# Zhen-Dong/HAWQ

Measured on AMD Instinct MI355X. Metric: images/sec, higher is better.
Workload: dtype int8

## Files before the change

### hawq_amd/_lib.py

```python
from __future__ import annotations

import ctypes as C
import os

_HERE = os.path.dirname(os.path.abspath(__file__))
LIB_PATH = os.environ.get("HAWQ_LIB") or os.path.join(_HERE, "lib", "libhawq_mi355.so")

EPI_RAW, EPI_REQUANT, EPI_RESIDUAL, EPI_DEQUANT = 0, 1, 2, 3

i32, i64, f32, vp = C.c_int32, C.c_int64, C.c_float, C.c_void_p


class ConvArgs(C.Structure):
    _fields_ = [
        ("in_", vp), ("wgt", vp), ("bias", vp),
        ("N", i32), ("H", i32), ("W", i32), ("Cin", i32), ("Cout", i32), ("KH", i32), ("KW", i32),
        ("stride", i32), ("pad", i32), ("in_bits", i32), ("w_bits", i32),
        ("in2", vp), ("wgt2", vp), ("bias2", vp),
        ("H2", i32), ("W2", i32), ("Cin2", i32), ("stride2", i32), ("in2_bits", i32), ("w2_bits", i32),
        ("epilogue", i32), ("relu", i32),
        ("m", vp), ("e", vp), ("m_id", vp), ("e_id", vp),
        ("m_id_scalar", i32), ("e_id_scalar", i32),
        ("res_in", vp), ("res_in_bits", i32),
        ("res_out", vp), ("res_out_bits", i32),
        ("out_q", vp), ("out_bits", i32), ("q_lo", i32), ("q_hi", i32), ("mq", i32), ("eq", i32),
        ("out_acc", vp), ("out_f32", vp), ("fscale", vp), ("ldo", i32), ("n_valid", i32),
        ("flags", vp), ("tile", i32), ("ctab", vp), ("ctab_id", vp), ("fast_tables", i32),
        ("in_planar", i32), ("out_planar", i32),
        ("res_no_relu", i32), ("res_clamp16", i32),
        ("in_pitch", i32), ("out_pitch", i32),
        ("wgt_band", vp), ("wgt_k128", vp), ("wgt2_k128", vp),
    ]


class ExpandReduceArgs(C.Structure):
    _fields_ = [("expand", ConvArgs), ("reduce", ConvArgs), ("tile", i32)]


class BottleneckArgs(C.Structure):
    _fields_ = [("expand", ConvArgs), ("project", ConvArgs), ("dw_wgt9c", vp), ("dw_ctab", vp),
                ("dw_stride", i32), ("dw_q_lo", i32), ("dw_q_hi", i32), ("dw_fast_tables", i32), ("c_mid", i32), ("tile", i32)]


class IncepConvArgs(C.Structure):
    _fields_ = [
        ("in_", vp), ("wgt", vp), ("bias", vp),
        ("N", i32), ("H", i32), ("W", i32), ("Cin", i32), ("Cout", i32), ("KH", i32), ("KW", i32),
        ("stride", i32), ("pad_h", i32), ("pad_w", i32),
        ("epilogue", i32), ("relu", i32),
        ("m", vp), ("ek", vp),
        ("q_lo", i32), ("q_hi", i32), ("m2", i32), ("ek2", i32), ("q2_lo", i32), ("q2_hi", i32),
        ("out", vp),
        ("out_bits", i32), ("ldo", i32), ("c_off", i32), ("reserved", i32),
    ]


INCEP_RAW, INCEP_REQUANT, INCEP_REQUANT2 = 0, 1, 2
INCEP_GROUP_MAX = 8


class IncepGroupArgs(C.Structure):
    _fields_ = [("n", i32), ("reserved", i32), ("conv", IncepConvArgs * INCEP_GROUP_MAX)]


INCEP_POOL_OPS = {"hawq_incep_requant": 0, "hawq_incep_maxpool3s2": 1, "hawq_incep_avgpool_branch": 2, "hawq_incep_global_avgpool": 3}


class IncepPoolArgs(C.Structure):
    _fields_ = [("in_", vp), ("out", vp)] + [(n, i32) for n in (
        "N", "H", "W", "C", "in_bits", "in_pitch", "in_off", "out_bits", "ldo", "c_off",
        "pre", "m1", "ek1", "lo1", "hi1", "post", "m2", "ek2", "lo2", "hi2")]


SIGNATURES = {
    "hawq_abi_version": [],
    "hawq_device_ok": [],
    "hawq_conv2d": [C.POINTER(ConvArgs), vp],
    "hawq_conv2d_num_tiles": [],
    "hawq_conv2d_num_band_tiles": [],
    "hawq_conv2d_band_tile": [C.POINTER(ConvArgs)],
    "hawq_conv2d_num_band2_tiles": [],
    "hawq_conv2d_band2_tile": [C.POINTER(ConvArgs)],
    "hawq_pack_w3x3_band": [vp, vp, i32, i32],
    "hawq_conv2d_num_gemm2_tiles": [],
    "hawq_conv2d_gemm2_first": [],
    "hawq_pack_w1x1_k128": [vp, vp, i32, i32],
    "hawq_conv2d_splitk_ok": [C.POINTER(ConvArgs), i32],
    "hawq_conv2d_splitk_workspace": [C.POINTER(ConvArgs), i32, C.POINTER(i64), C.POINTER(i64)],
    "hawq_conv2d_splitk": [C.POINTER(ConvArgs), i32, vp, vp, vp],
    "hawq_fc_dequant_ok": [i32, i32, i32],
    "hawq_fc_dequant": [vp, vp, vp, vp, vp, i32, i32, i32, i32, i32, vp],
    "hawq_conv_expand_reduce": [C.POINTER(ExpandReduceArgs), vp],
    "hawq_conv_expand_reduce_variants": [C.POINTER(ExpandReduceArgs)],
    "hawq_linear_bottleneck": [C.POINTER(BottleneckArgs), vp],
    "hawq_linear_bottleneck_ok": [C.POINTER(BottleneckArgs)],
    "hawq_stem3x3s2": [vp, vp, vp, i32, i32, f32, i32, i32, C.POINTER(ConvArgs), vp],
    "hawq_stem3x3s2_ok": [vp, vp, vp, i32, i32, C.POINTER(ConvArgs)],
    "hawq_quantize_input": [vp, vp, i32, i32, i32, i32, i32, i32, i32, i32, f32, i32, i32, vp],
    "hawq_stem_conv7": [vp, vp, vp, vp, vp, i32, i32, i32, i32, i32, i32, i32, vp, vp, vp],
    "hawq_stem_fused": [vp, i32, i32, i32, i32, f32, i32, i32, vp, vp, vp, vp, i32, i32, vp, vp, i32, i32, i32, i32, i32,
                        i32, vp],
    "hawq_stem_fused_u8": [vp, vp, i32, i32, i32, i32, vp, vp, vp, vp, i32, i32, vp, vp, i32, i32, i32, i32, i32, i32, vp],
    "hawq_maxpool3s2_requant": [vp, i32, i32, i32, i32, vp, vp, i32, i32, i32, i32, i32, vp],
    "hawq_requant_residual": [vp, i32, i64, vp, i32, i32, i32, i32, i32, vp],
    "hawq_avgpool_requant": [vp, i32, i32, i32, i32, vp, vp, i32, i32, i32, i32, vp],
    "hawq_f32_nchw_to_q_nhwc": [vp, vp, i32, i32, i32, i32, i32, i32, f32, vp],
    "hawq_acc_nhwc_to_f32_nchw": [vp, vp, i32, i32, i32, i32, i32, vp, vp],
    "hawq_fixedpoint_f32": [vp, vp, i32, i32, i32, f32, vp, vp, vp, i32, vp, f32, vp, vp, vp, i32, f32, i32, i32,
                            i32, vp],
    "hawq_fakequant_f32": [vp, vp, i64, f32, f32, i32, i32, vp],
    "hawq_avgpool_f32": [vp, vp, i32, i32, f32, vp],
    "hawq_conv2d_grouped": [vp, vp, vp, i32, i32, i32, i32, i32, i32, i32, i32, i32, i32, vp, vp],
    "hawq_depthwise3x3": [vp, vp, vp, i32, i32, i32, i32, i32, vp, vp],
    "hawq_depthwise3x3_requant": [vp, vp, vp, vp, vp, i32, i32, i32, i32, i32, i32, i32, i32, i32, vp, vp, vp],
# ... 77 lines not shown
```

### hawq_amd/csrc/conv_igemm.hip

```cpp
#include <stdio.h>
#include <stdlib.h>

#include "common.h"

namespace {

struct ConvP {
    const uint8_t *in, *wgt;
    const int32_t *bias;
    int N, H, W, Cin, Cout, KH, KW, stride, pad, Ho, Wo, M;
    int in_bits, w_bits;
    const uint8_t *in2, *wgt2;
    const int32_t *bias2;
    int H2, W2, Cin2, stride2, in2_bits, w2_bits;
    int relu;
    const int32_t *m, *e, *m_id, *e_id;
    int m_id_s, e_id_s;
    const void *res_in;
    int res_in_bits;
    void *res_out;
    int res_out_bits;
    void *out_q;
    int out_bits, q_lo, q_hi, mq, eq;
    int32_t *out_acc;
    float *out_f32;
    const float *fscale;
    int ldo, n_valid;
    int32_t *flags;
    const int32_t *ctab, *ctab_id;
    int k0;
    int ck0;
    int res_no_relu, res_clamp16;
    int ring_bytes;
    int in_planar, out_planar;
    int gfast;
    int in_pitch, out_pitch;
    int dbg;
    long long *dbgbuf;
};

template <int BM_, int BN_, int WM_, int WN_, int NS_, int KSUB_ = 1, int MINB_ = 2, int KG_ = 1>
struct Cfg {
    static constexpr int BM = BM_, BN = BN_, WM = WM_, WN = WN_;
    static constexpr int MINB = MINB_;
    static constexpr int NS = NS_;
    static constexpr int KSUB = KSUB_;
    static constexpr int KG = KG_;
    static constexpr int NWG = WM_ * WN_;
    static constexpr int NW = NWG * KG;
    static constexpr int NT = NW * 64;
    static constexpr int NTG = NWG * 64;
    static constexpr int RPP = NTG / 4;
    static constexpr int PT = BM / WM / 32;
    static constexpr int CT = BN / WN / 32;
    static constexpr int AL = BM / RPP;
    static constexpr int WL = BN / RPP;
    static constexpr int STAGE_BYTES = KSUB * (BM + BN) * 64;
    static constexpr int LDS_BYTES = NS * STAGE_BYTES;
    static_assert(NW == 4 || NW == 8 || NW == 16, "4, 8 or 16 waves per workgroup");
    static_assert(BM % RPP == 0 && BN % RPP == 0, "tile rows must fill whole staging passes");
    static_assert(KSUB % KG == 0 && (KG == 1 || BM * BN * 4 <= LDS_BYTES), "split-K: sub-chunks per group, partial sums staged on the ring");
};

template <bool SIGNED16>
__device__ __forceinline__ v4i unpack16(unsigned x0, unsigned x1) {
    v4i r;
    if (SIGNED16) {
        r.x = (int)((x0 << 4) & 0xF0F0F0F0u);
        r.y = (int)(x0 & 0xF0F0F0F0u);
        r.z = (int)((x1 << 4) & 0xF0F0F0F0u);
        r.w = (int)(x1 & 0xF0F0F0F0u);
    } else {
        r.x = (int)(x0 & 0x0F0F0F0Fu);
        r.y = (int)((x0 >> 4) & 0x0F0F0F0Fu);
        r.z = (int)(x1 & 0x0F0F0F0Fu);
        r.w = (int)((x1 >> 4) & 0x0F0F0F0Fu);
    }
    return r;
}

template <int BITS>
__device__ __forceinline__ v4i load_chunk16(const uint8_t *p, bool valid) {
    v4i z = {0, 0, 0, 0};
    if (!valid) return z;
    if (BITS == 8) return *reinterpret_cast<const v4i *>(p);
    v2i t = *reinterpret_cast<const v2i *>(p);
    z.x = t.x;
    z.y = t.y;
    return z;
}

template <class C, int A_BITS, int W_BITS>
__device__ __forceinline__ void gemm_segment(v16i (&acc)[C::CT][C::PT], const uint8_t *__restrict__ in,
                                             const uint8_t *__restrict__ wgt, int H, int W, int Cin, int KH,
                                             int KW, int stride, int pad, int Ho, int Wo, int M, int Cout,
                                             int m0, int c0, char *smem, int apitch) {
    const int t = threadIdx.x;
    const int lane = t & 63, wave = t >> 6;
    const int wave_m = wave % C::WM, wave_c = wave / C::WM;
    const int lrow = t >> 2, lslot = t & 3;
    constexpr int ABYTES = A_BITS == 8 ? 16 : 8;
    constexpr int WBYTES = W_BITS == 8 ? 16 : 8;

    int pix_base[C::AL], iy0[C::AL], ix0[C::AL];
    bool mval[C::AL];
#pragma unroll
    for (int i = 0; i < C::AL; ++i) {
        const int m = m0 + lrow + C::RPP * i;
        mval[i] = m < M;
        const int mm = mval[i] ? m : 0;
        const int n = mm / (Ho * Wo);
        const int r = mm - n * (Ho * Wo);
        const int oy = r / Wo, ox = r - oy * Wo;
        iy0[i] = oy * stride - pad;
        ix0[i] = ox * stride - pad;
        pix_base[i] = (n * H + iy0[i]) * W + ix0[i];
    }
    const int taps = KH * KW;
    const int cchunks = Cin >> 6;
// ... 232 lines not shown
                }
                return;
            }
            const int slot = 2 * (s & 1) + h;
#pragma unroll
            for (int c = 0; c < C::CT; ++c) wf[buf][c] = *reinterpret_cast<const v4i *>(ldsW + lds_off(wrow[c], slot));
#pragma unroll
            for (int q = 0; q < C::PT; ++q) af[buf][q] = *reinterpret_cast<const v4i *>(ldsA + lds_off(arow[q], slot));
        };
        constexpr int NOWN = SPS * KSUB / C::KG;
        auto step_of = [&](int o) { return C::KG == 1 ? o : ((o / SPS) * C::KG + kg) * SPS + (o % SPS); };
        fetch(step_of(0), 0);
#pragma unroll
        for (int o = 0; o < NOWN; ++o) {
            if (o + 1 < NOWN) fetch(step_of(o + 1), (o + 1) & 1);
#pragma unroll
            for (int c = 0; c < C::CT; ++c)
#pragma unroll
                for (int q = 0; q < C::PT; ++q)
                    a[c][q] = __builtin_amdgcn_mfma_i32_32x32x32_i8(wf[o & 1][c], af[o & 1][q], a[c][q], 0, 0, 0);
        }
    };

    const int ns1 = nk1 / KSUB, nst = RANGE ? ke : nk / KSUB;
    const int kfirst = RANGE ? kb : 0;
#pragma unroll
    for (int j = 0; j < NS - 1; ++j)
        if (kfirst + j < nst) issue();
    int cstage = 0;
    constexpr int LS = L * KSUB / C::KG;
    auto step = [&](auto &a, int k) {
        const int after = min(NS - 2, nst - 1 - k);
        if (after >= NS - 2) {
            wait_vmcnt<(NS - 2) * LS>();
        } else {
            switch (after) {
                case 5: wait_vmcnt<(NS > 6 ? 5 : 0) * LS>(); break;
                case 4: wait_vmcnt<(NS > 5 ? 4 : 0) * LS>(); break;
                case 3: wait_vmcnt<(NS > 4 ? 3 : 0) * LS>(); break;
                case 2: wait_vmcnt<(NS > 3 ? 2 : 0) * LS>(); break;
                case 1: wait_vmcnt<(NS > 2 ? 1 : 0) * LS>(); break;
                default: wait_vmcnt<0>(); break;
            }
        }
        __builtin_amdgcn_s_barrier();
        if (jissue < (RANGE ? nst * KSUB : nk) && !HAWQ_DBG_BIT(p.dbg, 1)) issue();
        if (!HAWQ_DBG_BIT(p.dbg, 2)) compute(a, cstage);
        if (++cstage == NS) cstage = 0;
    };
    for (int k = kfirst; k < (RANGE ? min(ns1, nst) : ns1); ++k) step(acc, k);
    if constexpr (DUAL)
        for (int k = RANGE ? max(ns1, kfirst) : ns1; k < nst; ++k) step(acc2, k);
    if constexpr (NIB) {
#pragma unroll
        for (int c = 0; c < C::CT; ++c)
#pragma unroll
            for (int q = 0; q < C::PT; ++q)
#pragma unroll
                for (int r = 0; r < 16; ++r) {
                    acc[c][q][r] >>= 4;
                    if constexpr (DUAL) acc2[DUAL ? c : 0][DUAL ? q : 0][r] >>= 4;
                }
    }
    __syncthreads();
}

template <class C, int BITS>
__device__ __forceinline__ void run_segment(v16i (&acc)[C::CT][C::PT], const uint8_t *in, const uint8_t *wgt,
                                            int a_bits, int w_bits, int H, int W, int Cin, int KH, int KW,
                                            int stride, int pad, int Ho, int Wo, int M, int Cout, int m0, int c0,
                                            char *smem, int apitch) {
    if (BITS == 0x88 || (BITS == 0 && a_bits == 8 && w_bits == 8))
        gemm_segment<C, 8, 8>(acc, in, wgt, H, W, Cin, KH, KW, stride, pad, Ho, Wo, M, Cout, m0, c0, smem, apitch);
    else if (BITS == 0x44 || (BITS == 0 && a_bits == 4 && w_bits == 4))
        gemm_segment<C, 4, 4>(acc, in, wgt, H, W, Cin, KH, KW, stride, pad, Ho, Wo, M, Cout, m0, c0, smem, apitch);
    else if (BITS == 0x84 || (BITS == 0 && a_bits == 8 && w_bits == 4))
        gemm_segment<C, 8, 4>(acc, in, wgt, H, W, Cin, KH, KW, stride, pad, Ho, Wo, M, Cout, m0, c0, smem, apitch);
    else
        gemm_segment<C, 4, 8>(acc, in, wgt, H, W, Cin, KH, KW, stride, pad, Ho, Wo, M, Cout, m0, c0, smem, apitch);
}

__device__ __forceinline__ v4i ld4(const int32_t *p) { return *reinterpret_cast<const v4i *>(p); }


template <class C, int EPI, bool DUAL>
__device__ __forceinline__ void epilogue_generic(const ConvP &p, v16i (&acc)[C::CT][C::PT],
                                                 v16i (&acc2)[DUAL ? C::CT : 1][DUAL ? C::PT : 1], int m0, int c0) {
    const int lane = threadIdx.x & 63, wave = threadIdx.x >> 6;
    const int wave_m = wave % C::WM, wave_c = wave / C::WM;
    const int l31 = lane & 31, h = lane >> 5;
#pragma unroll
    for (int c = 0; c < C::CT; ++c) {
        const int ch = c0 + wave_c * (C::CT * 32) + c * 32 + h * 16;
#pragma unroll
        for (int q = 0; q < C::PT; ++q) {
            const int pix = m0 + wave_m * (C::PT * 32) + q * 32 + l31;
            if (pix >= p.M) continue;
            constexpr bool PITCHED = EPI == HAWQ_EPI_REQUANT || EPI == HAWQ_EPI_RESIDUAL;
            const int opitch = PITCHED ? p.out_pitch : p.Cout;
            const size_t elem = (size_t)pix * opitch + ch;
            bool ovf = false;
            int qw[4] = {0, 0, 0, 0};
#pragma unroll
            for (int g = 0; g < 4; ++g) {
                if (PITCHED && ch + 4 * g >= opitch) continue;
                const v4i b4 = ld4(p.bias + ch + 4 * g);
                const int bb[4] = {b4.x, b4.y, b4.z, b4.w};
                int v[4], qv[4] = {0, 0, 0, 0}, o[4] = {0, 0, 0, 0};
#pragma unroll
                for (int j = 0; j < 4; ++j) v[j] = acc[c][q][4 * g + j] + bb[j];
                if constexpr (EPI == HAWQ_EPI_RAW) {
                    v4i w = {v[0], v[1], v[2], v[3]};
                    reinterpret_cast<v4i *>(p.out_acc + elem)[g] = w;
                } else if constexpr (EPI == HAWQ_EPI_DEQUANT) {
#pragma unroll
                    for (int j = 0; j < 4; ++j)
                        if (ch + 4 * g + j < p.n_valid)
                            p.out_f32[(size_t)pix * p.ldo + ch + 4 * g + j] = (float)v[j] * p.fscale[ch + 4 * g + j];
                } else if (p.n_valid > 0 && ch + 4 * g >= p.n_valid) {
                    if (EPI == HAWQ_EPI_RESIDUAL && p.res_out) {
                        if (p.res_out_bits == 16) reinterpret_cast<v2i *>((uint16_t *)p.res_out + elem)[g] = v2i{0, 0};
                        else reinterpret_cast<v4i *>((int32_t *)p.res_out + elem)[g] = v4i{0, 0, 0, 0};
                    }
                    if ((EPI == HAWQ_EPI_REQUANT || p.out_q) && p.out_bits == 4 && !(g & 1)) reinterpret_cast<uint32_t *>((uint8_t *)p.out_q + (elem >> 1) + (g >> 1) * 4)[0] = 0u;
                } else if (EPI == HAWQ_EPI_RESIDUAL && !DUAL && p.gfast) {
                    const bool tie = p.k0 == 2;
                    const DyNt dids = dynt_prepare(p.m_id_s, p.e_id_s), dq = dynt_prepare(p.mq, p.eq);
#pragma unroll
                    for (int j = 0; j < 4; ++j) {
                        const v4i t4 = ld4(p.ctab + (size_t)(ch + 4 * g + j) * 4);
                        DyNt dm;
                        dm.m = t4.x, dm.s = t4.y & 31, dm.k = t4.y >> 8;
                        dm.add = (long long)(((unsigned long long)(unsigned)t4.w << 32) | (unsigned)t4.z);
                        const int av = acc[c][q][4 * g + j];
                        int ov = tie ? dyadic_tie(av, dm) : dyadic_nt(av, dm);
                        if (p.res_in) {
                            const int r = p.res_in_bits == 16 ? (int)((const uint16_t *)p.res_in)[elem + 4 * g + j]
                                                              : ((const int32_t *)p.res_in)[elem + 4 * g + j];
                            ov += tie ? dyadic_tie(r, dids) : dyadic_nt(r, dids);
                        }
                        if (!p.res_no_relu) ov = max(ov, 0);
                        if (p.res_clamp16) ov = clampi(ov, -32768, 32767);
                        o[j] = ov;
                        qv[j] = clampi(tie ? dyadic_tie(ov, dq) : dyadic_nt(ov, dq), p.q_lo, p.q_hi);
                        ovf |= ov > 65535;
                    }
                    if (p.res_out) {
                        if (p.res_out_bits == 16) {
                            v2i w = {min(o[0], 65535) | (min(o[1], 65535) << 16), min(o[2], 65535) | (min(o[3], 65535) << 16)};
                            reinterpret_cast<v2i *>((uint16_t *)p.res_out + elem)[g] = w;
                        } else {
                            v4i w = {o[0], o[1], o[2], o[3]};
                            reinterpret_cast<v4i *>((int32_t *)p.res_out + elem)[g] = w;
                        }
                    }
                    if (p.out_q) {
                        if (p.out_bits == 8) {
                            qw[g] = (int)pack4_i8(qv[0], qv[1], qv[2], qv[3]);
                        } else {
                            uint8_t *dst = (uint8_t *)p.out_q + (elem >> 1) + (g >> 1) * 4;
#pragma unroll
                            for (int j = 0; j < 4; ++j) dst[j] = (g & 1) ? (uint8_t)((dst[j] & 0x0f) | (qv[j] << 4)) : (uint8_t)(qv[j] & 0x0f);
                        }
                    }
                } else {
                    const v4i m4 = ld4(p.m + ch + 4 * g), e4 = ld4(p.e + ch + 4 * g);
                    const int mm[4] = {m4.x, m4.y, m4.z, m4.w}, ee[4] = {e4.x, e4.y, e4.z, e4.w};
                    if constexpr (EPI == HAWQ_EPI_REQUANT) {
#pragma unroll
                        for (int j = 0; j < 4; ++j)
                            qv[j] = clampi(dyadic_rne(p.relu ? max(v[j], 0) : v[j], mm[j], ee[j]), p.q_lo, p.q_hi);
                    } else {
                        int idv[4];
                        if constexpr (DUAL) {
                            const v4i b2 = ld4(p.bias2 + ch + 4 * g), mi = ld4(p.m_id + ch + 4 * g),
                                      ei = ld4(p.e_id + ch + 4 * g);
                            const int bb2[4] = {b2.x, b2.y, b2.z, b2.w}, m1[4] = {mi.x, mi.y, mi.z, mi.w},
                                      e1[4] = {ei.x, ei.y, ei.z, ei.w};
#pragma unroll
                            for (int j = 0; j < 4; ++j) idv[j] = dyadic_rne(acc2[DUAL ? c : 0][DUAL ? q : 0][4 * g + j] + bb2[j], m1[j], e1[j]);
                        } else if (p.res_in) {
#pragma unroll
                            for (int j = 0; j < 4; ++j) {
                                const int r = p.res_in_bits == 16 ? (int)((const uint16_t *)p.res_in)[elem + 4 * g + j]
                                                                  : ((const int32_t *)p.res_in)[elem + 4 * g + j];
                                idv[j] = dyadic_rne(r, p.m_id_s, p.e_id_s);
                            }
                        } else {
#pragma unroll
                            for (int j = 0; j < 4; ++j) idv[j] = 0;
                        }
#pragma unroll
                        for (int j = 0; j < 4; ++j) {
                            o[j] = dyadic_rne(v[j], mm[j], ee[j]) + idv[j];
                            if (!p.res_no_relu) o[j] = max(o[j], 0);
                            if (p.res_clamp16) o[j] = clampi(o[j], -32768, 32767);
                            qv[j] = clampi(dyadic_rne(o[j], p.mq, p.eq), p.q_lo, p.q_hi);
                            ovf |= o[j] > 65535;
                        }
                        if (p.res_out) {
                            if (p.res_out_bits == 16) {
                                v2i w = {min(o[0], 65535) | (min(o[1], 65535) << 16), min(o[2], 65535) | (min(o[3], 65535) << 16)};
                                reinterpret_cast<v2i *>((uint16_t *)p.res_out + elem)[g] = w;
                            } else {
                                v4i w = {o[0], o[1], o[2], o[3]};
                                reinterpret_cast<v4i *>((int32_t *)p.res_out + elem)[g] = w;
                            }
                        }
                    }
                    if (EPI == HAWQ_EPI_REQUANT || p.out_q) {
                        if (p.out_bits == 8) {
                            qw[g] = (int)pack4_i8(qv[0], qv[1], qv[2], qv[3]);
                        } else {
                            uint8_t *dst = (uint8_t *)p.out_q + (elem >> 1) + (g >> 1) * 4;
                            if (g & 1) {
#pragma unroll
                                for (int j = 0; j < 4; ++j) dst[j] = (uint8_t)((dst[j] & 0x0f) | (qv[j] << 4));
                            } else {
#pragma unroll
                                for (int j = 0; j < 4; ++j) dst[j] = (uint8_t)(qv[j] & 0x0f);
                            }
                        }
                    }
                }
            }
            if constexpr (PITCHED) {
                if ((EPI == HAWQ_EPI_REQUANT || p.out_q) && p.out_bits == 8 && ch < opitch)
                    *reinterpret_cast<v4i *>((char *)p.out_q + elem) = v4i{qw[0], qw[1], qw[2], qw[3]};
            }
            if (EPI == HAWQ_EPI_RESIDUAL && ovf && p.res_out && p.res_out_bits == 16) atomicOr(p.flags, 1);
        }
    }
}

template <class C>
struct Stage {
    static constexpr int RCPR = C::BN / 8;
    static constexpr int QCPR = C::BN / 16;
    __device__ static __forceinline__ int rsw(int row) { return row & (RCPR - 1); }
    __device__ static __forceinline__ int qsw(int row) {
        return QCPR >= 8 ? (row & (QCPR - 1)) : ((row >> 1) & (QCPR - 1));
    }
};

template <class C>
__device__ __forceinline__ void prefetch_residual(const ConvP &p, int m0, int c0, char *res_tile) {
    using S = Stage<C>;
    const int wave = threadIdx.x >> 6, lane = threadIdx.x & 63;
#pragma unroll
    for (int i = 0; i < (C::BM * S::RCPR + C::NT - 1) / C::NT; ++i) {
        const int base = (i * C::NW + wave) * 64;
        if (base >= C::BM * S::RCPR) break;
        const int idx = base + lane;
        const int row = idx / S::RCPR, j = idx % S::RCPR;
        const int grow = (m0 + row < p.M) ? m0 + row : m0;
        const char *src = (const char *)p.res_in + ((size_t)grow * p.Cout + c0) * 2 + ((j ^ S::rsw(row)) << 4);
        __builtin_amdgcn_global_load_lds((const __attribute__((address_space(1))) void *)src,
                                         (__attribute__((address_space(3))) void *)(res_tile + base * 16), 16, 0, 0);
    }
}

template <class C, int EPI, bool DUAL, int MODE = 0, bool CK0 = false>
__device__ __forceinline__ void epilogue_fast(const ConvP &p, v16i (&acc)[C::CT][C::PT],
                                              v16i (&acc2)[DUAL ? C::CT : 1][DUAL ? C::PT : 1], int m0, int c0,
                                              char *q_tile, char *res_tile, const char *ctab_lds,
                                              const bool active = true) {
    using S = Stage<C>;
    constexpr bool RES = EPI == HAWQ_EPI_RESIDUAL;
    constexpr bool K0 = MODE == 1 || CK0;
    constexpr int MODE_C = (CK0 && MODE == 0) ? 1 : MODE;
    const int lane = threadIdx.x & 63, wave = threadIdx.x >> 6;
    const int wave_m = wave % C::WM, wave_c = (wave / C::WM) % C::WN;
    const int l31 = lane & 31, h = lane >> 5;
    const int lrow0 = wave_m * (C::PT * 32) + l31;
    DyNt dids = dynt_prepare(p.m_id_s, p.e_id_s), dq = dynt_prepare(p.mq, p.eq);
    asm volatile("" : "+s"(dids.add), "+s"(dq.add));
    const int qhi2 = (p.q_hi & 0xffff) | (p.q_hi << 16);
    unsigned oor = 0;
    unsigned rowmask[C::PT];
#pragma unroll
    for (int q = 0; q < C::PT; ++q) rowmask[q] = (m0 + lrow0 + q * 32 < p.M) ? 0xffffffffu : 0u;
    if (active)
#pragma unroll
    for (int c = 0; c < C::CT; ++c) {
        const int lch = wave_c * (C::CT * 32) + c * 32 + h * 16;
        constexpr int WPS = (C::NT / 256 > C::MINB) ? C::NT / 256 : C::MINB;
        constexpr int QPASS = (DUAL || (RES && WPS >= 4)) ? C::PT : 1, QPER = C::PT / QPASS;
#pragma unroll
        for (int qp = 0; qp < QPASS; ++qp) {
        v4i rin[C::PT][2];
        if constexpr (RES && !DUAL) {
#pragma unroll
            for (int qq = 0; qq < QPER; ++qq) {
                const int q = qp * QPER + qq;
                const int row = lrow0 + q * 32;
                const char *base = res_tile + row * (S::RCPR * 16);
                rin[q][0] = *reinterpret_cast<const v4i *>(base + (((lch >> 3) ^ S::rsw(row)) << 4));
                rin[q][1] = *reinterpret_cast<const v4i *>(base + ((((lch >> 3) + 1) ^ S::rsw(row)) << 4));
            }
        }
        int qpack[QPER][4];
        int rpack[QPER][RES ? 8 : 1];
#pragma unroll
        for (int g = 0; g < 4; ++g) {
            DyNt dm[4], di[4];
#pragma unroll
            for (int j = 0; j < 4; ++j) {
                const v4i t = *reinterpret_cast<const v4i *>(ctab_lds + (lch + 4 * g + j) * 16);
                dm[j].m = t.x, dm[j].s = K0 ? t.y : (t.y & 31), dm[j].k = K0 ? 0 : (t.y >> 8);
                dm[j].add = (long long)(((unsigned long long)(unsigned)t.w << 32) | (unsigned)t.z);
                if constexpr (DUAL) {
                    const v4i u = *reinterpret_cast<const v4i *>(ctab_lds + C::BN * 16 + (lch + 4 * g + j) * 16);
                    di[j].m = u.x, di[j].s = K0 ? u.y : (u.y & 31), di[j].k = K0 ? 0 : (u.y >> 8);
                    di[j].add = (long long)(((unsigned long long)(unsigned)u.w << 32) | (unsigned)u.z);
                } else {
                    di[j] = dids;
                }
            }
#pragma unroll
            for (int qq = 0; qq < QPER; ++qq) {
                const int q = qp * QPER + qq;
                int qv[4];
                if constexpr (!RES) {
#pragma unroll
                    for (int j = 0; j < 4; ++j)
                        qv[j] = med3i(dyadic_mode<MODE_C>(acc[c][q][4 * g + j], dm[j]), p.q_lo, p.q_hi);
                } else {
                    int idin[4], o[4];
                    if constexpr (DUAL) {
#pragma unroll
                        for (int j = 0; j < 4; ++j) idin[j] = acc2[DUAL ? c : 0][DUAL ? q : 0][4 * g + j];
                    } else {
                        const unsigned w0 = (unsigned)rin[q][g >> 1][(g & 1) * 2], w1 = (unsigned)rin[q][g >> 1][(g & 1) * 2 + 1];
                        idin[0] = (int)(w0 & 0xffffu), idin[1] = (int)(w0 >> 16);
                        idin[2] = (int)(w1 & 0xffffu), idin[3] = (int)(w1 >> 16);
                    }
#pragma unroll
                    for (int j = 0; j < 4; ++j) {
                        const int a = dyadic_mode<MODE_C>(acc[c][q][4 * g + j], dm[j]);
// ... 441 lines not shown
        BAND_FETCH(0, 0)
        for (int s = 0; s < nsteps; ++s) {
            BAND_BATCH(0)
            if (C::NPROD == 0 && early && !HAWQ_DBG_BIT(p.dbg, 1)) issue_step(s, cc, kh);
            BAND_BATCH(1)
            BAND_BATCH(2)
            BAND_BATCH(3)
            if (C::NPROD == 0 && !early && !HAWQ_DBG_BIT(p.dbg, 1)) issue_step(s, cc, kh);
            BAND_BATCH(4)
            if (++kh == 3) kh = 0, ++cc;
            if (s + 1 < nsteps) {
                bases(s + 1, cc, kh);
                BAND_FETCH(0, 0)
                wait_lgkm<C::CT + C::PT>();
            } else {
                wait_lgkm<0>();
            }
            BAND_MMA(5)
            if (C::NPROD == 0) wait_vmcnt<0>();
            __builtin_amdgcn_s_barrier();
        }
#undef BAND_FETCH
#undef BAND_MMA
#undef BAND_BATCH
        if (C::NPROD > 0) __builtin_amdgcn_s_setprio(0);
    }
    const long long t_loop_end = prof ? (long long)__builtin_readcyclecounter() : 0;
    if constexpr (NIB) {
#pragma unroll
        for (int c = 0; c < C::CT; ++c)
#pragma unroll
            for (int q = 0; q < C::PT; ++q)
#pragma unroll
                for (int r = 0; r < 16; ++r) acc[c][q][r] >>= 4;
    }
    __syncthreads();
    if constexpr (EPI == HAWQ_EPI_RESIDUAL) {
        using S = Stage<C>;
        static_assert(C::BM * C::BN * 2 <= C::WS * C::WSTAGE && C::BM * C::BN <= C::BSTAGES * C::BAND_BYTES, "epilogue tiles alias the rings");
        constexpr int NWALL = C::NT / 64, PPW = C::BM * S::RCPR / 64 / NWALL;
        static_assert(PPW * NWALL * 64 == C::BM * S::RCPR, "residual tile pieces");
#pragma unroll
        for (int i = 0; i < PPW; ++i) {
            const int base = (i * NWALL + wave) * 64, idx = base + lane;
            const int row = idx / S::RCPR, j = idx % S::RCPR;
            const int grow = (m0 + row < p.M) ? m0 + row : m0;
            const char *src = (const char *)p.res_in + ((size_t)grow * p.Cout + c0) * 2 + ((j ^ S::rsw(row)) << 4);
            __builtin_amdgcn_global_load_lds((const __attribute__((address_space(1))) void *)src,
                                             (__attribute__((address_space(3))) void *)(wring + base * 16), 16, 0, 0);
        }
        wait_vmcnt<0>();
        __syncthreads();
    }
    v16i dummy[1][1];
    epilogue_fast<C, EPI, false, TIE ? 2 : 0>(p, acc, dummy, m0, c0, smem, wring, ctab_lds, consumer);
    if (prof && blockIdx.x == 8 && t == 0) {
        p.dbgbuf[0] = t_begin - t_entry, p.dbgbuf[1] = t_loop_end - t_begin;
        p.dbgbuf[2] = (long long)__builtin_readcyclecounter() - t_loop_end, p.dbgbuf[3] = nsteps;
    }
}

using B0 = BandCfg<256, 64, 4, 1, 512, 1, 2, 0>;
using B1 = BandCfg<256, 128, 4, 2, 512, 2, 1, 8>;
using B2 = BandCfg<128, 128, 2, 4, 256, 2, 1, 8, 4>;
using B3 = BandCfg<256, 128, 4, 2, 384, 2, 1, 8, 4>;
using B4 = BandCfg<128, 128, 2, 4, 256, 2, 1, 8, 5>;
using B5 = BandCfg<128, 64, 2, 2, 256, 2, 4, 4, 3>;
constexpr int NUM_BAND_TILES = 6;

typedef void (*KernelFn)(const ConvP);
struct BandInfo { KernelFn fn[2][2][2]; int bm, bn, band_px, bstages, lds, nt; };
#define BAND_FN(B, N, T) {conv3x3_band_kernel<B, N, T, HAWQ_EPI_REQUANT>, conv3x3_band_kernel<B, N, T, HAWQ_EPI_RESIDUAL>}
#define BAND_ENTRY(B) {{{BAND_FN(B, false, false), BAND_FN(B, false, true)}, {BAND_FN(B, true, false), BAND_FN(B, true, true)}}, B::BM, B::BN, B::BAND_PX, B::BSTAGES, B::LDS_BYTES + B::BN * 16, B::NT}
const BandInfo kBand[NUM_BAND_TILES] = {BAND_ENTRY(B0), BAND_ENTRY(B1), BAND_ENTRY(B2), BAND_ENTRY(B3), BAND_ENTRY(B4), BAND_ENTRY(B5)};
const int kBandPreference[NUM_BAND_TILES] = {0, 3, 1, 2, 4, 5};

bool band_applies(const BandInfo &bi, const hawq_conv_args *a) {
    const int wo = a->W, band_rows = (bi.bm + wo - 1) / wo + 1 + 2;
    const bool nib = a->in_bits == 4 && a->w_bits == 4;
    const bool res = a->epilogue == HAWQ_EPI_RESIDUAL;
    const bool epi_ok = (a->epilogue == HAWQ_EPI_REQUANT && a->out_q) ||
                        (res && a->res_in && a->res_in_bits == 16 && (!a->res_out || a->res_out_bits == 16));
    const bool dense = (a->in_pitch == 0 || a->in_pitch == a->Cin * a->in_bits / 8) && (a->out_pitch == 0 || a->out_pitch == a->Cout);
    return a->KH == 3 && a->KW == 3 && a->stride == 1 && a->pad == 1 && a->in2 == nullptr && a->fast_tables != 0 && epi_ok && dense &&
           ((a->in_bits == 8 && a->w_bits == 8) || (nib && a->Cin % 128 == 0)) && a->Cout % bi.bn == 0 &&
           band_rows * (wo + 2) <= bi.band_px - 4 && (bi.bstages > 1 || (a->Cin >> (nib ? 7 : 6)) == 1);
}

using T0 = Cfg<128, 128, 2, 2, 3>;
using T1 = Cfg<256, 64, 4, 1, 3>;
using T2 = Cfg<64, 64, 2, 2, 4>;
using T3 = Cfg<128, 64, 2, 2, 4>;
using T4 = Cfg<128, 128, 2, 2, 3, 2>;
using T5 = Cfg<64, 64, 2, 2, 4, 2>;
using T6 = Cfg<128, 64, 2, 2, 3, 2>;
using T7 = Cfg<128, 128, 2, 4, 3>;
using T8 = Cfg<128, 128, 2, 4, 3, 2>;
using T9 = Cfg<256, 128, 4, 2, 3>;
using T10 = Cfg<64, 64, 2, 2, 3, 1, 6>;
using T11 = Cfg<64, 64, 2, 2, 2, 1, 6>;
using T12 = Cfg<128, 64, 2, 2, 2, 1, 3>;
using T13 = Cfg<128, 128, 2, 4, 2, 1, 2>;
using T14 = Cfg<64, 64, 2, 2, 3, 2, 4, 2>;
constexpr int NUM_TILES = 15;

struct TileInfo {
    int BM, BN, lds, ksub, twin, nt, ns, kg;
    KernelFn single[4][3];
    KernelFn dual[5];
    KernelFn tie_single[2][2];
    KernelFn tie_dual[2];
};
#define SINGLE_ROW(T, E) \
    { conv_kernel<T, E, false, 0, 0>, conv_kernel<T, E, false, 0x88, 0>, conv_kernel<T, E, false, 0x44, 0> }
#define TILE_ENTRY(T, TWIN)                                                                                          \
    {                                                                                                          \
        T::BM, T::BN, T::LDS_BYTES, T::KSUB, TWIN, T::NT, T::NS, T::KG,                                                   \
            {SINGLE_ROW(T, HAWQ_EPI_RAW), SINGLE_ROW(T, HAWQ_EPI_REQUANT), SINGLE_ROW(T, HAWQ_EPI_RESIDUAL),   \
             SINGLE_ROW(T, HAWQ_EPI_DEQUANT)},                                                                 \
        {                                                                                                      \
            conv_kernel<T, HAWQ_EPI_RESIDUAL, true, 0, 0>, conv_kernel<T, HAWQ_EPI_RESIDUAL, true, 0x88, 0x88>, \
                conv_kernel<T, HAWQ_EPI_RESIDUAL, true, 0x44, 0x44>,                                           \
                conv_kernel<T, HAWQ_EPI_RESIDUAL, true, 0x88, 0x44>,                                           \
                conv_kernel<T, HAWQ_EPI_RESIDUAL, true, 0x44, 0x88>                                            \
        },                                                                                                     \
        {{conv_kernel<T, HAWQ_EPI_REQUANT, false, 0x88, 0, true>, conv_kernel<T, HAWQ_EPI_REQUANT, false, 0x44, 0, true>},   \
         {conv_kernel<T, HAWQ_EPI_RESIDUAL, false, 0x88, 0, true>, conv_kernel<T, HAWQ_EPI_RESIDUAL, false, 0x44, 0, true>}}, \
        {conv_kernel<T, HAWQ_EPI_RESIDUAL, true, 0x88, 0x88, true>, conv_kernel<T, HAWQ_EPI_RESIDUAL, true, 0x44, 0x44, true>} \
    }
const TileInfo kTiles[NUM_TILES] = {TILE_ENTRY(T0, 0), TILE_ENTRY(T1, 1), TILE_ENTRY(T2, 2), TILE_ENTRY(T3, 3),
                                    TILE_ENTRY(T4, 0), TILE_ENTRY(T5, 2), TILE_ENTRY(T6, 3),
                                    TILE_ENTRY(T7, 7), TILE_ENTRY(T8, 7), TILE_ENTRY(T9, 9),
                                    TILE_ENTRY(T10, 10), TILE_ENTRY(T11, 11), TILE_ENTRY(T12, 12), TILE_ENTRY(T13, 13),
                                    TILE_ENTRY(T14, 2)};

bool raise_lds_limits() {
    bool ok = true;
    for (const TileInfo &ti : kTiles) {
        const int lds = ti.lds + ti.BM * ti.BN * 2 + ti.BN * 32;
        if (lds <= 64 * 1024) continue;
        for (int v = 0; v < 2; ++v)
            ok &= hipFuncSetAttribute((const void *)ti.tie_single[1][v], hipFuncAttributeMaxDynamicSharedMemorySize, lds) == hipSuccess &&
                  hipFuncSetAttribute((const void *)ti.tie_dual[v], hipFuncAttributeMaxDynamicSharedMemorySize, lds) == hipSuccess;
        for (int v = 1; v < 3; ++v)
            ok &= hipFuncSetAttribute((const void *)ti.single[2][v], hipFuncAttributeMaxDynamicSharedMemorySize, lds) ==
                  hipSuccess;
        for (int v = 1; v < 5; ++v)
            ok &= hipFuncSetAttribute((const void *)ti.dual[v], hipFuncAttributeMaxDynamicSharedMemorySize, lds) ==
                  hipSuccess;
    }
    return ok;
}

int pick_tile(int M, int Cout, bool dual) {
    auto nwg = [&](int t) { return ((M + kTiles[t].BM - 1) / kTiles[t].BM) * (Cout / kTiles[t].BN); };
    if (dual) return nwg(3) >= 512 ? 3 : 2;
    if (Cout % 128 == 0 && nwg(0) >= 1024) return 0;
    if (nwg(1) >= 1024 && !dual) return 1;
    if (Cout % 128 == 0 && nwg(0) >= 512) return 0;
    if (nwg(3) >= 512) return 3;
    return 2;
}

#endif
}
#ifndef HAWQ_CONV_IGEMM_DEVICE_ONLY

bool band_persist_applies(const hawq_conv_args *a);
int band_persist_launch(const hawq_conv_args *a, int exact_tie, int dbg, int wgs_per_cu, void *stream);

int gemm_v2_count(void);
bool gemm_v2_applies(const hawq_conv_args *a, int v);
int gemm_v2_launch(const hawq_conv_args *a, int v, int exact_tie, int dbg, void *stream);
int band_v2_count(void);
bool band_v2_applies(const hawq_conv_args *a, int v);
int band_v2_launch(const hawq_conv_args *a, int v, int exact_tie, int dbg, void *stream);

extern "C" int hawq_conv2d_num_tiles(void) { return NUM_TILES + NUM_BAND_TILES + 2 + band_v2_count() + gemm_v2_count(); }
extern "C" int hawq_conv2d_num_gemm2_tiles(void) { return gemm_v2_count(); }
extern "C" int hawq_conv2d_gemm2_first(void) { return NUM_TILES + NUM_BAND_TILES + 2 + band_v2_count() + 1; }
extern "C" int hawq_conv2d_num_band_tiles(void) { return NUM_BAND_TILES + 2 + band_v2_count() + gemm_v2_count(); }

extern "C" int hawq_conv2d_num_band2_tiles(void) { return band_v2_count(); }
extern "C" int hawq_conv2d_band2_tile(const hawq_conv_args *a) {
    if (!a || a->W <= 0 || a->H <= 0 || a->Cin <= 0 || a->Cout <= 0) return 0;
    for (int v = 0; v < band_v2_count(); ++v)
        if (band_v2_applies(a, v)) return NUM_TILES + NUM_BAND_TILES + 2 + v + 1;
    return 0;
}

extern "C" int hawq_conv2d_band_tile(const hawq_conv_args *a) {
    if (!a || a->W <= 0 || a->H <= 0 || a->Cin <= 0 || a->Cout <= 0) return 0;
    for (int k = 0; k < NUM_BAND_TILES; ++k)
        if (band_applies(kBand[kBandPreference[k]], a)) return NUM_TILES + kBandPreference[k] + 1;
    return 0;
}

extern "C" int hawq_conv2d(const hawq_conv_args *a, void *stream) {
    HAWQ_REQUIRE(a != nullptr, "hawq_conv2d: null args");
    HAWQ_REQUIRE(a->in && a->wgt && a->bias, "hawq_conv2d: in/wgt/bias must be non-null");
    HAWQ_REQUIRE(a->Cin > 0 && a->Cin % 64 == 0, "hawq_conv2d: Cin=%d must be a positive multiple of 64", a->Cin);
    HAWQ_REQUIRE(a->Cout > 0 && a->Cout % 64 == 0, "hawq_conv2d: Cout=%d must be a positive multiple of 64", a->Cout);
    HAWQ_REQUIRE((a->in_bits == 8 || a->in_bits == 4) && (a->w_bits == 8 || a->w_bits == 4),
                 "hawq_conv2d: in_bits/w_bits must be 4 or 8 (got %d/%d)", a->in_bits, a->w_bits);
    HAWQ_REQUIRE(a->KH > 0 && a->KW > 0 && a->stride > 0 && a->pad >= 0 && a->N > 0 && a->H > 0 && a->W > 0,
                 "hawq_conv2d: bad geometry");
    ConvP p;
    p.in = (const uint8_t *)a->in;
    p.wgt = (const uint8_t *)a->wgt;
    p.bias = a->bias;
    p.N = a->N, p.H = a->H, p.W = a->W, p.Cin = a->Cin, p.Cout = a->Cout;
    p.KH = a->KH, p.KW = a->KW, p.stride = a->stride, p.pad = a->pad;
    p.Ho = (a->H + 2 * a->pad - a->KH) / a->stride + 1;
    p.Wo = (a->W + 2 * a->pad - a->KW) / a->stride + 1;
    HAWQ_REQUIRE(p.Ho > 0 && p.Wo > 0, "hawq_conv2d: empty output");
    const long long M = (long long)a->N * p.Ho * p.Wo;
    HAWQ_REQUIRE(M * (long long)a->Cout < (1ll << 40) && M < (1ll << 30), "hawq_conv2d: problem too large");
    p.M = (int)M;
    p.in_bits = a->in_bits, p.w_bits = a->w_bits;
    const bool dual = a->in2 != nullptr;
    p.in2 = (const uint8_t *)a->in2, p.wgt2 = (const uint8_t *)a->wgt2, p.bias2 = a->bias2;
    p.H2 = a->H2, p.W2 = a->W2, p.Cin2 = a->Cin2, p.stride2 = a->stride2;
    p.in2_bits = a->in2_bits, p.w2_bits = a->w2_bits;
    if (dual) {
        HAWQ_REQUIRE(a->epilogue == HAWQ_EPI_RESIDUAL, "hawq_conv2d: second branch needs HAWQ_EPI_RESIDUAL");
        HAWQ_REQUIRE(a->wgt2 && a->bias2 && a->m_id && a->e_id, "hawq_conv2d: second branch tables missing");
        HAWQ_REQUIRE(a->Cin2 > 0 && a->Cin2 % 64 == 0, "hawq_conv2d: Cin2 must be a multiple of 64");
        HAWQ_REQUIRE((a->in2_bits == 8 || a->in2_bits == 4) && (a->w2_bits == 8 || a->w2_bits == 4),
                     "hawq_conv2d: in2_bits/w2_bits must be 4 or 8");
        HAWQ_REQUIRE((a->H2 - 1) / a->stride2 + 1 == p.Ho && (a->W2 - 1) / a->stride2 + 1 == p.Wo,
                     "hawq_conv2d: second branch output grid differs");
    }
    p.relu = a->relu;
    p.m = a->m, p.e = a->e, p.m_id = a->m_id, p.e_id = a->e_id;
    p.m_id_s = a->m_id_scalar, p.e_id_s = a->e_id_scalar;
    p.res_in = a->res_in, p.res_in_bits = a->res_in_bits;
    p.res_no_relu = a->res_no_relu, p.res_clamp16 = a->res_clamp16;
    p.res_out = a->res_out, p.res_out_bits = a->res_out_bits;
    p.out_q = a->out_q, p.out_bits = a->out_bits, p.q_lo = a->q_lo, p.q_hi = a->q_hi, p.mq = a->mq, p.eq = a->eq;
    p.out_acc = a->out_acc, p.out_f32 = a->out_f32, p.fscale = a->fscale, p.ldo = a->ldo, p.n_valid = a->n_valid;
    {
        const int dense_in = a->Cin * a->in_bits / 8;
        p.in_pitch = a->in_pitch ? a->in_pitch : dense_in, p.out_pitch = a->out_pitch ? a->out_pitch : a->Cout;
        if (p.in_pitch != dense_in)
            HAWQ_REQUIRE(a->in_pitch > 0 && a->in_pitch % 16 == 0 && a->in_pitch < dense_in && a->in_bits == 8 && !a->in_planar,
                         "hawq_conv2d: in_pitch=%d needs a multiple of 16 below the dense row (%d bytes), int8 activations, NHWC rows", a->in_pitch, dense_in);
        if (p.out_pitch != a->Cout) {
            const bool fast_ = a->fast_tables != 0;
            HAWQ_REQUIRE(a->out_pitch > 0 && a->out_pitch % 16 == 0 && a->out_pitch < a->Cout, "hawq_conv2d: out_pitch=%d needs a multiple of 16 below Cout=%d", a->out_pitch, a->Cout);
            HAWQ_REQUIRE((a->epilogue == HAWQ_EPI_REQUANT || a->epilogue == HAWQ_EPI_RESIDUAL) && !a->in2 && !a->out_planar && (!a->out_q || a->out_bits == 8),
                         "hawq_conv2d: out_pitch exists for single-branch REQUANT / RESIDUAL launches with int8 NHWC outputs");
            const bool direct_ = a->epilogue == HAWQ_EPI_RESIDUAL &&
                                 (a->res_no_relu || a->res_clamp16 || !a->res_in || a->res_in_bits == 32 || (a->res_out && a->res_out_bits == 32));
            HAWQ_REQUIRE(!fast_ || a->epilogue == HAWQ_EPI_REQUANT || direct_,
                         "hawq_conv2d: out_pitch with fast_tables needs the REQUANT epilogue or a signed / 32-bit RESIDUAL (the unsigned 16-bit fast RESIDUAL tiles are dense)");
            HAWQ_REQUIRE(a->n_valid <= a->out_pitch, "hawq_conv2d: n_valid=%d exceeds out_pitch=%d", a->n_valid, a->out_pitch);
        }
    }
    p.flags = a->flags;
    p.ctab = a->ctab, p.ctab_id = a->ctab_id;
    static const int dbg_env = HAWQ_DBG_ENV();
    p.dbg = a->fast_tables ? dbg_env : 0;
    p.dbgbuf = nullptr;
    static long long *dbg_dev = nullptr;
    if (HAWQ_DBG_BIT(p.dbg, 128) && !dbg_dev) (void)hipMalloc(&dbg_dev, 64 * sizeof(long long));
    if (HAWQ_DBG_BIT(p.dbg, 128)) p.dbgbuf = dbg_dev;
    const bool fast = a->fast_tables != 0;
    p.k0 = (a->fast_tables & 4) ? 2 : ((a->fast_tables & 2) ? 1 : 0);
    p.ck0 = (a->fast_tables & 8) != 0;
    if (fast && (a->epilogue == HAWQ_EPI_REQUANT || a->epilogue == HAWQ_EPI_RESIDUAL)) {
        HAWQ_REQUIRE(a->ctab && (!dual || a->ctab_id), "hawq_conv2d: fast_tables needs ctab (and ctab_id)");
        if (a->epilogue == HAWQ_EPI_REQUANT && a->relu && p.q_lo < 0) p.q_lo = 0;
        const bool direct_form = a->epilogue == HAWQ_EPI_RESIDUAL && !dual &&
                                 (a->res_no_relu || a->res_clamp16 || !a->res_in || a->res_in_bits == 32 || (a->res_out && a->res_out_bits == 32));
        HAWQ_REQUIRE(a->epilogue != HAWQ_EPI_RESIDUAL || !a->out_q || a->q_lo <= 0 || direct_form,
                     "hawq_conv2d: fast RESIDUAL needs q_lo <= 0");
    }
    auto e_fast = [](int ek) { return (ek & 0xff) >= 33 && (ek & 0xff) <= 62; };
    auto e_any = [](int ek) { return (ek & 0xff) >= 1 && (ek & 0xff) <= 62 && (ek >> 8) >= 0 && (ek >> 8) < 31; };
    if (a->epilogue == HAWQ_EPI_RESIDUAL) {
        if (a->out_q) {
            HAWQ_REQUIRE(a->mq >= 0 && e_any(a->eq), "hawq_conv2d: bad (mq, eq)");
            HAWQ_REQUIRE(!fast || e_fast(a->eq), "hawq_conv2d: fast_tables needs eq in [33,62]");
            HAWQ_REQUIRE(!fast || (a->q_hi >= 0 && a->q_hi <= 32767), "hawq_conv2d: fast_tables needs 0 <= q_hi <= 32767 for the next QuantAct");
            HAWQ_REQUIRE(p.k0 != 1 || (a->eq >> 8) == 0, "hawq_conv2d: fast_tables bit 1 (no pre-shifts) but eq carries one");
        } else {
            p.mq = 0, p.eq = 33;
        }
        if (!dual && !a->res_in) {
            p.m_id_s = 0, p.e_id_s = 33;
        } else if (!dual) {
            HAWQ_REQUIRE(a->m_id_scalar >= 0 && e_any(a->e_id_scalar), "hawq_conv2d: bad (m_id_scalar, e_id_scalar)");
            HAWQ_REQUIRE(!fast || e_fast(a->e_id_scalar), "hawq_conv2d: fast_tables needs e_id_scalar in [33,62]");
        } else {
            p.m_id_s = 0, p.e_id_s = 33;
        }
    } else {
        p.mq = 0, p.eq = 33, p.m_id_s = 0, p.e_id_s = 33;
    }
    int slot = -1;
// ... 155 lines not shown
```

### hawq_amd/csrc/conv_splitk.hip

```cpp
#define HAWQ_CONV_IGEMM_DEVICE_ONLY
#include "conv_igemm.hip"

namespace {

using SK = Cfg<64, 64, 2, 2, 4>;
constexpr int SK_TILE = SK::BM * SK::BN;
constexpr int SK_RES = SK::BM * SK::BN * 2;
constexpr int SK_CTAB = SK::BN * 16 * 2;
constexpr int SK_LDS = SK::LDS_BYTES + SK_RES + SK_CTAB + 16;

struct SplitP {
    int32_t *slab;
    int32_t *counters;
    int tiles_c, ntiles;
    int s1, s2;
    int q1, q2;
    int ns1;
};

template <int EPI, bool DUAL, bool FAST, bool TIE, bool PLANAR>
__global__ __launch_bounds__(SK::NT, SK::MINB) void conv_splitk_kernel(const ConvP p, const SplitP s) {
    using C = SK;
    extern __shared__ __attribute__((aligned(16))) char smem[];
    const int tile = blockIdx.x % s.ntiles, z = blockIdx.x / s.ntiles;
// ... 3 lines not shown

    v16i acc[C::CT][C::PT], acc2[C::CT][C::PT];
#pragma unroll
    for (int r = 0; r < 16; ++r) acc[0][0][r] = 0;
    const int kb = z < s.s1 ? z * s.q1 : s.ns1 + (z - s.s1) * s.q2;
    const int ke = kb + (z < s.s1 ? s.q1 : s.q2);
    gemm_pipeline<C, DUAL, false, true, PLANAR>(acc, acc, p, m0, c0, smem, kb, ke);

    const size_t tile_base = (size_t)tile * nsl * SK_TILE;
    int32_t *mine = s.slab + tile_base + (size_t)z * SK_TILE + wave * 1024;
#pragma unroll
    for (int g = 0; g < 4; ++g)
        reinterpret_cast<v4i *>(mine)[g * 64 + lane] = v4i{acc[0][0][4 * g], acc[0][0][4 * g + 1], acc[0][0][4 * g + 2], acc[0][0][4 * g + 3]};
    __builtin_amdgcn_fence(__ATOMIC_RELEASE, "agent");
    __syncthreads();
    int *last = reinterpret_cast<int *>(smem + SK_LDS - 16);
    if (threadIdx.x == 0) {
        const int arrived = __hip_atomic_fetch_add(s.counters + tile, 1, __ATOMIC_RELAXED, __HIP_MEMORY_SCOPE_AGENT);
        *last = arrived == nsl - 1;
    }
    __syncthreads();
    if (!*last) return;
    __builtin_amdgcn_fence(__ATOMIC_ACQUIRE, "agent");
    if (threadIdx.x == 0) s.counters[tile] = 0;

#pragma unroll
    for (int r = 0; r < 16; ++r) acc[0][0][r] = 0, acc2[0][0][r] = 0;
    const int32_t *base = s.slab + tile_base + wave * 1024;
    for (int j = 0; j < s.s1; ++j) {
#pragma unroll
        for (int g = 0; g < 4; ++g) {
            const v4i v = reinterpret_cast<const v4i *>(base + (size_t)j * SK_TILE)[g * 64 + lane];
            acc[0][0][4 * g] += v.x, acc[0][0][4 * g + 1] += v.y, acc[0][0][4 * g + 2] += v.z, acc[0][0][4 * g + 3] += v.w;
        }
    }
    if constexpr (DUAL) {
        for (int j = s.s1; j < nsl; ++j) {
#pragma unroll
            for (int g = 0; g < 4; ++g) {
                const v4i v = reinterpret_cast<const v4i *>(base + (size_t)j * SK_TILE)[g * 64 + lane];
                acc2[0][0][4 * g] += v.x, acc2[0][0][4 * g + 1] += v.y, acc2[0][0][4 * g + 2] += v.z, acc2[0][0][4 * g + 3] += v.w;
            }
        }
    }

    if constexpr (FAST) {
        char *res_tile = smem + p.ring_bytes;
        char *ctab_lds = res_tile + (EPI == HAWQ_EPI_RESIDUAL ? SK_RES : 0);
        if (wave < C::BN / 64)
            __builtin_amdgcn_global_load_lds((const __attribute__((address_space(1))) void *)(p.ctab + (size_t)(c0 + wave * 64 + lane) * 4),
                                             (__attribute__((address_space(3))) void *)(ctab_lds + wave * 1024), 16, 0, 0);
        if constexpr (DUAL) {
            if (wave >= C::NW / 2 && wave - C::NW / 2 < C::BN / 64)
                __builtin_amdgcn_global_load_lds(
                    (const __attribute__((address_space(1))) void *)(p.ctab_id + (size_t)(c0 + (wave - C::NW / 2) * 64 + lane) * 4),
                    (__attribute__((address_space(3))) void *)(ctab_lds + C::BN * 16 + (wave - C::NW / 2) * 1024), 16, 0, 0);
        }
        if constexpr (EPI == HAWQ_EPI_RESIDUAL && !DUAL) prefetch_residual<C>(p, m0, c0, res_tile);
        wait_vmcnt<0>();
        __syncthreads();
        epilogue_fast<C, EPI, DUAL, TIE ? 2 : 0>(p, acc, acc2, m0, c0, smem, res_tile, ctab_lds);
    } else {
        epilogue_generic<C, EPI, DUAL>(p, acc, acc2, m0, c0);
    }
}

typedef void (*SplitFn)(const ConvP, const SplitP);

struct SplitPlan {
    int s1, s2, q1, q2, ns1, tiles_c, ntiles, M, Ho, Wo;
    long long slab_bytes, counter_bytes;
};

int splitk_plan(const hawq_conv_args *a, int slices, SplitPlan &sp) {
    HAWQ_REQUIRE(a != nullptr, "hawq_conv2d_splitk: null args");
    HAWQ_REQUIRE(slices >= 2, "hawq_conv2d_splitk: slices=%d (at least 2)", slices);
    HAWQ_REQUIRE(a->Cin > 0 && a->Cin % 64 == 0 && a->Cout > 0 && a->Cout % 64 == 0, "hawq_conv2d_splitk: Cin / Cout must be positive multiples of 64");
    HAWQ_REQUIRE(a->N > 0 && a->H > 0 && a->W > 0, "hawq_conv2d_splitk: bad geometry");
    HAWQ_REQUIRE(a->in_bits == 8 && a->w_bits == 8, "hawq_conv2d_splitk: int8 operands only (in_bits %d, w_bits %d)", a->in_bits, a->w_bits);
    const bool k1 = a->KH == 1 && a->KW == 1 && a->pad == 0, k3 = a->KH == 3 && a->KW == 3 && a->pad == 1;
    HAWQ_REQUIRE((k1 || k3) && (a->stride == 1 || a->stride == 2), "hawq_conv2d_splitk: 1x1 / pad 0 or 3x3 / pad 1 convs with stride 1 or 2 only");
    HAWQ_REQUIRE(a->n_valid == 0 && (a->in_pitch == 0 || a->in_pitch == a->Cin) && (a->out_pitch == 0 || a->out_pitch == a->Cout),
                 "hawq_conv2d_splitk: n_valid / in_pitch / out_pitch are not supported");
    const int epi = a->epilogue;
    HAWQ_REQUIRE(epi == HAWQ_EPI_RAW || epi == HAWQ_EPI_REQUANT || epi == HAWQ_EPI_RESIDUAL, "hawq_conv2d_splitk: RAW, REQUANT or RESIDUAL epilogue only");
    HAWQ_REQUIRE(epi == HAWQ_EPI_RAW || !a->out_q || a->out_bits == 8, "hawq_conv2d_splitk: out_bits must be 8");
    HAWQ_REQUIRE(epi != HAWQ_EPI_REQUANT || a->out_q, "hawq_conv2d_splitk: REQUANT needs out_q");
    HAWQ_REQUIRE((a->in_planar | a->out_planar | 1) == 1, "hawq_conv2d_splitk: in_planar / out_planar must be 0 or 1");
    const bool dual = a->in2 != nullptr;
    const bool fast = a->fast_tables != 0;
    const bool res = epi == HAWQ_EPI_RESIDUAL;
    const bool wide_res = res && ((!dual && a->res_in_bits == 32) || (a->res_out && a->res_out_bits == 32));
    const bool signed_res = res && !dual && (a->res_no_relu || a->res_clamp16 || !a->res_in);
    const bool fast_epi = fast && epi != HAWQ_EPI_RAW && !wide_res && !signed_res;
    HAWQ_REQUIRE(!a->in_planar || (!dual && fast_epi), "hawq_conv2d_splitk: in_planar needs a single-branch fast-contract REQUANT / RESIDUAL launch");
    HAWQ_REQUIRE(!a->out_planar || (fast_epi && a->out_q), "hawq_conv2d_splitk: out_planar needs the fast-contract REQUANT / RESIDUAL epilogue");
    sp.Ho = (a->H + 2 * a->pad - a->KH) / a->stride + 1;
    sp.Wo = (a->W + 2 * a->pad - a->KW) / a->stride + 1;
    const long long M = (long long)a->N * sp.Ho * sp.Wo;
    HAWQ_REQUIRE(sp.Ho > 0 && sp.Wo > 0 && M < (1ll << 30) && M * (long long)a->Cout < (1ll << 40), "hawq_conv2d_splitk: bad output size");
    sp.M = (int)M;
    const int nk1 = a->KH * a->KW * (a->Cin >> 6);
    HAWQ_REQUIRE(nk1 % slices == 0, "hawq_conv2d_splitk: %d slices do not divide the %d K chunks", slices, nk1);
    sp.s1 = slices, sp.q1 = nk1 / slices, sp.ns1 = nk1, sp.s2 = 0, sp.q2 = 1;
    if (dual) {
        HAWQ_REQUIRE(res, "hawq_conv2d_splitk: a second branch needs HAWQ_EPI_RESIDUAL");
        HAWQ_REQUIRE(a->in2_bits == 8 && a->w2_bits == 8, "hawq_conv2d_splitk: int8 operands only in the second branch");
        HAWQ_REQUIRE(a->Cin2 > 0 && a->Cin2 % 64 == 0 && a->stride2 > 0 && a->H2 > 0 && a->W2 > 0, "hawq_conv2d_splitk: bad second branch");
        HAWQ_REQUIRE((a->H2 - 1) / a->stride2 + 1 == sp.Ho && (a->W2 - 1) / a->stride2 + 1 == sp.Wo, "hawq_conv2d_splitk: second branch output grid differs");
        const int nk2 = a->Cin2 >> 6;
        int q2 = sp.q1 < nk2 ? sp.q1 : nk2;
        while (nk2 % q2) --q2;
        sp.q2 = q2, sp.s2 = nk2 / q2;
    }
    sp.tiles_c = a->Cout / SK::BN;
    sp.ntiles = ((sp.M + SK::BM - 1) / SK::BM) * sp.tiles_c;
    HAWQ_REQUIRE((long long)sp.ntiles * (sp.s1 + sp.s2) < (1ll << 31), "hawq_conv2d_splitk: grid too large");
    sp.slab_bytes = (long long)sp.ntiles * (sp.s1 + sp.s2) * SK_TILE * 4;
    sp.counter_bytes = (long long)sp.ntiles * 4;
    return 0;
}

#define SK_FN(E, D, F, T, P) conv_splitk_kernel<E, D, F, T, P>
SplitFn pick_kernel(int epi, bool dual, bool fast, bool tie, bool planar) {
    if (epi == HAWQ_EPI_RAW) return SK_FN(HAWQ_EPI_RAW, false, false, false, false);
    if (dual) {
        if (!fast) return SK_FN(HAWQ_EPI_RESIDUAL, true, false, false, false);
        return tie ? SK_FN(HAWQ_EPI_RESIDUAL, true, true, true, false) : SK_FN(HAWQ_EPI_RESIDUAL, true, true, false, false);
    }
    if (epi == HAWQ_EPI_REQUANT) {
        if (!fast) return SK_FN(HAWQ_EPI_REQUANT, false, false, false, false);
        if (planar) return tie ? SK_FN(HAWQ_EPI_REQUANT, false, true, true, true) : SK_FN(HAWQ_EPI_REQUANT, false, true, false, true);
        return tie ? SK_FN(HAWQ_EPI_REQUANT, false, true, true, false) : SK_FN(HAWQ_EPI_REQUANT, false, true, false, false);
    }
    if (!fast) return SK_FN(HAWQ_EPI_RESIDUAL, false, false, false, false);
    if (planar) return tie ? SK_FN(HAWQ_EPI_RESIDUAL, false, true, true, true) : SK_FN(HAWQ_EPI_RESIDUAL, false, true, false, true);
    return tie ? SK_FN(HAWQ_EPI_RESIDUAL, false, true, true, false) : SK_FN(HAWQ_EPI_RESIDUAL, false, true, false, false);
}

}

extern "C" int hawq_conv2d_splitk_ok(const hawq_conv_args *a, int32_t slices) {
    SplitPlan sp;
    return splitk_plan(a, slices, sp) == 0 ? 1 : 0;
}

extern "C" int hawq_conv2d_splitk_workspace(const hawq_conv_args *a, int32_t slices, int64_t *slab_bytes, int64_t *counter_bytes) {
    SplitPlan sp;
    const int rc = splitk_plan(a, slices, sp);
    if (rc) return rc;
    if (slab_bytes) *slab_bytes = sp.slab_bytes;
    if (counter_bytes) *counter_bytes = sp.counter_bytes;
    return 0;
}

extern "C" int hawq_conv2d_splitk(const hawq_conv_args *a, int32_t slices, void *slab, int32_t *counters, void *stream) {
    SplitPlan sp;
    const int rc = splitk_plan(a, slices, sp);
    if (rc) return rc;
    HAWQ_REQUIRE(slab && counters, "hawq_conv2d_splitk: slab and counters must be non-null");
    HAWQ_REQUIRE(a->in && a->wgt && a->bias, "hawq_conv2d_splitk: in/wgt/bias must be non-null");
    const bool dual = a->in2 != nullptr;
    const int epi = a->epilogue;
    const bool fast = a->fast_tables != 0;
    ConvP p = {};
    p.in = (const uint8_t *)a->in, p.wgt = (const uint8_t *)a->wgt, p.bias = a->bias;
// ... 65 lines not shown
```

### hawq_amd/csrc/fused_er.hip

```cpp
#include <stdio.h>
#include <stdlib.h>

#include "common.h"

namespace {

struct ERP {
    const uint8_t *x2, *w3, *w1;
    const uint8_t *xid, *wid;
    const int32_t *ctab3, *ctab1, *ctab_id;
    const uint16_t *res_in;
    uint16_t *res_out;
    uint8_t *y;
    int M, C3;
    int m_id_s, e_id_s, mq, eq, q_hi;
    int y_lo, y_hi;
    int y_planar;
    int y_nib;
    int32_t *flags;
    int dbg;
    long long *dbgbuf;
};

__device__ __attribute__((aligned(16))) const int g_er_zero16[4] = {0, 0, 0, 0};
// ... 298 lines not shown
            __syncthreads();
            if (p.y_planar) {
                for (int idx = t; idx < F::BM * CPN; idx += F::NTC) {
                    const int ch = idx / F::BM, row = idx % F::BM;
                    if (m0 + row < p.M)
                        *reinterpret_cast<v4i *>((char *)p.y + ((size_t)ch * p.M + (m0 + row)) * 16) =
                            *reinterpret_cast<const v4i *>(yt + (row * CPN + (ch ^ (row & (CPN - 1)))) * 16);
                }
            } else {
                for (int idx = t; idx < F::BM * CPN; idx += F::NTC) {
                    const int row = idx / CPN, jj = idx % CPN;
                    if (m0 + row < p.M)
                        *reinterpret_cast<v4i *>((char *)p.y + (size_t)(m0 + row) * (F::C / 2) + ((jj ^ (row & (CPN - 1))) << 4)) =
                            *reinterpret_cast<const v4i *>(yt + idx * 16);
                }
            }
            return;
        }
#pragma unroll
        for (int c = 0; c < F::CT2; ++c) {
            const int ch0 = wave_c * (F::CT2 * 32) + c * 32 + h * 16;
            int w[4];
#pragma unroll
            for (int g = 0; g < 4; ++g) {
                int qv[4];
#pragma unroll
                for (int k = 0; k < 4; ++k)
                    qv[k] = med3i(dyadic_mode<MODE_C>(acc2[c][4 * g + k], ctab_entry<K0>((const char *)p.ctab1, ch0 + 4 * g + k)), p.y_lo, p.y_hi);
                w[g] = pack4_fast(qv[0], qv[1], qv[2], qv[3]);
            }
            const v4i ww = {w[0], w[1], w[2], w[3]};
            *reinterpret_cast<v4i *>(yt + (arow * CPR + ((ch0 >> 4) ^ (arow & (CPR - 1)))) * 16) = ww;
        }
        __syncthreads();
        if (p.y_planar) {
#pragma unroll
            for (int i = 0; i < F::BM * CPR / F::NTC; ++i) {
                const int idx = t + F::NTC * i, ch = idx / F::BM, row = idx % F::BM;
                if (m0 + row < p.M)
                    *reinterpret_cast<v4i *>((char *)p.y + ((size_t)ch * p.M + (m0 + row)) * 16) =
                        *reinterpret_cast<const v4i *>(yt + (row * CPR + (ch ^ (row & (CPR - 1)))) * 16);
            }
        } else {
#pragma unroll
            for (int i = 0; i < F::BM * CPR / F::NTC; ++i) {
                const int idx = t + F::NTC * i, row = idx / CPR, jj = idx % CPR;
                if (m0 + row < p.M)
                    *reinterpret_cast<v4i *>((char *)p.y + (size_t)(m0 + row) * F::C + ((jj ^ (row & (CPR - 1))) << 4)) =
                        *reinterpret_cast<const v4i *>(yt + idx * 16);
            }
        }
    }
}

using E64 = ERCfg<64, 2, 0, true, 4>;
using E64R = ERCfg<64, 2, 0, false, 4>;
using E128 = ERCfg<128, 2, 0, false, 3>;
using E128D = ERCfg<128, 2, 0, true, 3>;
using E128P = ERCfg<128, 2, 4, true, 4>;
using E256 = ERCfg<256, 4, 0, false, 2>;
using E256P = ERCfg<256, 4, 4, true, 3>;
using E256S = ERCfg<256, 2, 0, false, 2>;
using E256SP = ERCfg<256, 2, 4, true, 2>;
using E64D = ERCfg<64, 2, 0, false, 4, true>;
constexpr int NUM_ER = 10;

typedef void (*ERFn)(const ERP);
struct ERInfo { ERFn fn[5]; int c, bm, nt, lds; bool dual; };
#define ER_ENTRY(F) {{expand_reduce_kernel<F, false>, expand_reduce_kernel<F, true>, expand_reduce_kernel<F, false, true>, expand_reduce_kernel<F, false, true, true>, \
                      expand_reduce_kernel<F, false, false, true>}, F::C, F::BM, F::NT, F::LDS_BYTES, F::DUAL}
const ERInfo kER[NUM_ER] = {ER_ENTRY(E64), ER_ENTRY(E64R), ER_ENTRY(E128), ER_ENTRY(E128D), ER_ENTRY(E128P), ER_ENTRY(E256), ER_ENTRY(E256P), ER_ENTRY(E256S), ER_ENTRY(E256SP), ER_ENTRY(E64D)};

bool conv_is_1x1_int8_fast(const hawq_conv_args &a, bool dual_ok = false) {
    return (a.in_pitch == 0 || a.in_pitch == a.Cin) && (a.out_pitch == 0 || a.out_pitch == a.Cout) && a.KH == 1 && a.KW == 1 && a.stride == 1 && a.pad == 0 && a.in_bits == 8 && a.w_bits == 8 && a.fast_tables != 0 &&
           (dual_ok || !a.in2) && !a.in_planar;
}

bool dual_branch_fits(const hawq_conv_args &e) {
    return e.in2 && e.wgt2 && e.ctab_id && e.Cin2 == e.Cin && e.stride2 == 1 && e.H2 == e.H && e.W2 == e.W && e.in2_bits == 8 && e.w2_bits == 8;
}

int er_variant(const hawq_expand_reduce_args *a) {
    const hawq_conv_args &e = a->expand, &r = a->reduce;
    if (!conv_is_1x1_int8_fast(e, true) || !conv_is_1x1_int8_fast(r)) return -1;
    const bool dual = e.in2 != nullptr;
    if (dual && !dual_branch_fits(e)) return -1;
    if (e.epilogue != HAWQ_EPI_RESIDUAL || r.epilogue != HAWQ_EPI_REQUANT) return -1;
    if (!dual && (!e.res_in || e.res_in_bits != 16)) return -1;
    if (!e.res_out || e.res_out_bits != 16 || !e.flags || !e.ctab || !r.ctab || !r.out_q) return -1;
    if ((r.out_bits != 8 && r.out_bits != 4) || e.out_bits != 8) return -1;
    if (r.out_bits == 4 && (r.q_lo < 0 || r.q_hi > 15)) return -1;
    if (r.Cin != e.Cout || r.Cout != e.Cin || r.N != e.N || r.H != e.H || r.W != e.W || e.Cout % 64) return -1;
    int nth = 0, first = -1;
    for (int i = 0; i < NUM_ER; ++i)
        if (kER[i].c == e.Cin && kER[i].dual == dual) {
            if (first < 0) first = i;
            if (++nth == a->tile) return i;
        }
    return a->tile == 0 ? first : -1;
}

}

int wp_num_variants(const hawq_expand_reduce_args *a);
int wp_launch(const hawq_expand_reduce_args *a, int nth, void *stream);
int er2_num_variants(const hawq_expand_reduce_args *a);
int er2_launch(const hawq_expand_reduce_args *a, int nth, void *stream);

namespace {
int er_count(const hawq_expand_reduce_args *a) {
    if (!a->reduce.wgt) return 0;
    hawq_expand_reduce_args q = *a;
    q.tile = 0;
    if (er_variant(&q) < 0) return 0;
    int n = 0;
    for (int i = 0; i < NUM_ER; ++i) n += kER[i].c == a->expand.Cin && kER[i].dual == (a->expand.in2 != nullptr);
    return n;
}
}

extern "C" int hawq_conv_expand_reduce_variants(const hawq_expand_reduce_args *a) {
    if (!a) return 0;
    return er_count(a) + wp_num_variants(a) + er2_num_variants(a);
}

extern "C" int hawq_conv_expand_reduce(const hawq_expand_reduce_args *a, void *stream) {
    HAWQ_REQUIRE(a != nullptr, "hawq_conv_expand_reduce: null args");
    const int n_er = er_count(a), n_wp = wp_num_variants(a);
    if (a->tile > n_er + n_wp) return er2_launch(a, a->tile - n_er - n_wp, stream);
    if (a->tile > n_er || (a->tile == 0 && n_er == 0)) return wp_launch(a, a->tile == 0 ? 1 : a->tile - n_er, stream);
    const int v = er_variant(a);
    HAWQ_REQUIRE(v >= 0, "hawq_conv_expand_reduce: this pair of layers cannot be fused (need 1x1/stride-1 int8 fast-contract convs, "
                         "uint16 residual in and out - or a same-shape 1x1 identity branch with Cin 64 -, Cin in {64,128,256}, reduce.Cin == expand.Cout, reduce.Cout == expand.Cin; tile %d)", a->tile);
    const hawq_conv_args &e = a->expand, &r = a->reduce;
    auto e_fast = [](int ek) { return (ek & 0xff) >= 33 && (ek & 0xff) <= 62; };
    HAWQ_REQUIRE(e.mq >= 0 && e_fast(e.eq) && (e.in2 || (e.m_id_scalar >= 0 && e_fast(e.e_id_scalar))), "hawq_conv_expand_reduce: scalar tables outside the fast contract");
    HAWQ_REQUIRE(e.q_lo <= 0, "hawq_conv_expand_reduce: the block-input QuantAct clamp must admit 0");
    ERP p;
    p.x2 = (const uint8_t *)e.in, p.w3 = (const uint8_t *)e.wgt, p.w1 = (const uint8_t *)r.wgt;
    p.ctab3 = e.ctab, p.ctab1 = r.ctab;
    p.xid = (const uint8_t *)e.in2, p.wid = (const uint8_t *)e.wgt2, p.ctab_id = e.ctab_id;
    p.res_in = (const uint16_t *)e.res_in, p.res_out = (uint16_t *)e.res_out;
    p.y = (uint8_t *)r.out_q;
    const long long M = (long long)e.N * e.H * e.W;
    HAWQ_REQUIRE(M > 0 && M < (1ll << 30), "hawq_conv_expand_reduce: bad problem size");
    p.M = (int)M, p.C3 = e.Cout;
    p.m_id_s = e.in2 ? 0 : e.m_id_scalar, p.e_id_s = e.in2 ? 33 : e.e_id_scalar, p.mq = e.mq, p.eq = e.eq, p.q_hi = e.q_hi;
    p.y_lo = r.relu && r.q_lo < 0 ? 0 : r.q_lo, p.y_hi = r.q_hi;
    p.y_planar = r.out_planar;
    p.y_nib = r.out_bits == 4;
    p.flags = e.flags;
    static const int dbg_env = HAWQ_DBG_ENV();
    static long long *dbg_dev = nullptr;
    if (HAWQ_DBG_BIT(dbg_env, 128) && !dbg_dev) (void)hipMalloc(&dbg_dev, 64 * sizeof(long long));
    p.dbgbuf = HAWQ_DBG_BIT(dbg_env, 128) ? dbg_dev : nullptr;
    p.dbg = dbg_env;
    const ERInfo &ei = kER[v];
    static const bool attrs = [] {
        bool good = true;
        for (const ERInfo &k : kER)
            for (int i = 0; i < 5; ++i)
                good &= hipFuncSetAttribute((const void *)k.fn[i], hipFuncAttributeMaxDynamicSharedMemorySize, k.lds) == hipSuccess;
        return good;
    }();
    HAWQ_REQUIRE(attrs, "hawq_conv_expand_reduce: hipFuncSetAttribute(MaxDynamicSharedMemorySize) failed");
    const bool tie = ((e.fast_tables | r.fast_tables) & 4) != 0, ck0 = (e.fast_tables & 8) && (r.fast_tables & 8);
    const bool qk0 = (e.eq >> 8) == 0;
// ... 14 lines not shown
```

### hawq_amd/csrc/fused_er2.hip

```cpp
#include <stdio.h>
#include <stdlib.h>

#include "common.h"

namespace {

struct E2P {
    const uint8_t *x2, *w3, *w1;
    const int32_t *ctab3, *ctab1;
    const uint16_t *res_in;
    uint16_t *res_out;
    uint8_t *y;
    int M, C3;
    int m_id_s, e_id_s, mq, eq, q_hi;
    int y_lo, y_hi;
    int y_planar, y_nib;
    int32_t *flags;
    long long *dbgbuf;
    int dbg;
};

__device__ __attribute__((aligned(16))) const int g_e2_zero16[4] = {0, 0, 0, 0};

template <int C_, int WM_, int NP_, int MINB_, int SG_ = 4>
// ... 260 lines not shown
            constexpr int CPN = F::C / 32;
#pragma unroll
            for (int c = 0; c < F::CT2; ++c) {
                const int ch0 = wave_c * (F::CT2 * 32) + c * 32 + h * 16;
                int qv[16];
#pragma unroll
                for (int k = 0; k < 16; ++k)
                    qv[k] = med3i(dyadic_mode<MODE_C>(acc2[c][k], e2_ctab_entry<K0>((const char *)p.ctab1, ch0 + k)), p.y_lo, p.y_hi);
                const v2i ww = {(int)pack8_u4(&qv[0]), (int)pack8_u4(&qv[8])};
                *reinterpret_cast<v2i *>(yt + (arow * CPN + ((ch0 >> 5) ^ (arow & (CPN - 1)))) * 16 + ((ch0 >> 4) & 1) * 8) = ww;
            }
            __syncthreads();
            if (p.y_planar) {
                for (int idx = t; idx < F::BM * CPN; idx += F::NTC) {
                    const int ch = idx / F::BM, row = idx % F::BM;
                    if (m0 + row < p.M)
                        *reinterpret_cast<v4i *>((char *)p.y + ((size_t)ch * p.M + (m0 + row)) * 16) =
                            *reinterpret_cast<const v4i *>(yt + (row * CPN + (ch ^ (row & (CPN - 1)))) * 16);
                }
            } else {
                for (int idx = t; idx < F::BM * CPN; idx += F::NTC) {
                    const int row = idx / CPN, jj = idx % CPN;
                    if (m0 + row < p.M)
                        *reinterpret_cast<v4i *>((char *)p.y + (size_t)(m0 + row) * (F::C / 2) + ((jj ^ (row & (CPN - 1))) << 4)) =
                            *reinterpret_cast<const v4i *>(yt + idx * 16);
                }
            }
            return;
        }
#pragma unroll
        for (int c = 0; c < F::CT2; ++c) {
            const int ch0 = wave_c * (F::CT2 * 32) + c * 32 + h * 16;
            int w[4];
#pragma unroll
            for (int g = 0; g < 4; ++g) {
                int qv[4];
#pragma unroll
                for (int k = 0; k < 4; ++k)
                    qv[k] = med3i(dyadic_mode<MODE_C>(acc2[c][4 * g + k], e2_ctab_entry<K0>((const char *)p.ctab1, ch0 + 4 * g + k)), p.y_lo, p.y_hi);
                w[g] = pack4_fast(qv[0], qv[1], qv[2], qv[3]);
            }
            const v4i ww = {w[0], w[1], w[2], w[3]};
            *reinterpret_cast<v4i *>(yt + (arow * CPR + ((ch0 >> 4) ^ (arow & (CPR - 1)))) * 16) = ww;
        }
        __syncthreads();
        if (p.y_planar) {
#pragma unroll
            for (int i = 0; i < F::BM * CPR / F::NTC; ++i) {
                const int idx = t + F::NTC * i, ch = idx / F::BM, row = idx % F::BM;
                if (m0 + row < p.M)
                    *reinterpret_cast<v4i *>((char *)p.y + ((size_t)ch * p.M + (m0 + row)) * 16) =
                        *reinterpret_cast<const v4i *>(yt + (row * CPR + (ch ^ (row & (CPR - 1)))) * 16);
            }
        } else {
#pragma unroll
            for (int i = 0; i < F::BM * CPR / F::NTC; ++i) {
                const int idx = t + F::NTC * i, row = idx / CPR, jj = idx % CPR;
                if (m0 + row < p.M)
                    *reinterpret_cast<v4i *>((char *)p.y + (size_t)(m0 + row) * F::C + ((jj ^ (row & (CPR - 1))) << 4)) =
                        *reinterpret_cast<const v4i *>(yt + idx * 16);
            }
        }
    }
}

using P256B = E2Cfg<256, 4, 4, 3, 2>;
using P128A = E2Cfg<128, 4, 8, 4>;
using P128B = E2Cfg<128, 2, 4, 4>;
using P64A = E2Cfg<64, 4, 4, 3>;
constexpr int NUM_E2 = 4;

typedef void (*E2Fn)(const E2P);
struct E2Info { E2Fn fn[5]; int c, bm, nt, lds; };
#define E2_ENTRY(F) {{expand_reduce_pipelined_kernel<F, false>, expand_reduce_pipelined_kernel<F, true>, expand_reduce_pipelined_kernel<F, false, true>, \
                      expand_reduce_pipelined_kernel<F, false, true, true>, expand_reduce_pipelined_kernel<F, false, false, true>}, F::C, F::BM, F::NT, F::LDS_BYTES}
const E2Info kE2[NUM_E2] = {E2_ENTRY(P256B), E2_ENTRY(P128A), E2_ENTRY(P128B), E2_ENTRY(P64A)};

bool e2_conv_ok(const hawq_conv_args &a) {
    return (a.in_pitch == 0 || a.in_pitch == a.Cin) && (a.out_pitch == 0 || a.out_pitch == a.Cout) && a.KH == 1 && a.KW == 1 && a.stride == 1 && a.pad == 0 && a.in_bits == 8 && a.w_bits == 8 && a.fast_tables != 0 && !a.in2 && !a.in_planar;
}

int e2_variant(const hawq_expand_reduce_args *a, int nth) {
    const hawq_conv_args &e = a->expand, &r = a->reduce;
    if (!r.wgt || !e2_conv_ok(e) || !e2_conv_ok(r)) return -1;
    if (e.epilogue != HAWQ_EPI_RESIDUAL || r.epilogue != HAWQ_EPI_REQUANT) return -1;
    if (!e.res_in || e.res_in_bits != 16 || !e.res_out || e.res_out_bits != 16 || !e.flags || !e.ctab || !r.ctab || !r.out_q) return -1;
    if ((r.out_bits != 8 && r.out_bits != 4) || e.out_bits != 8) return -1;
    if (r.out_bits == 4 && (r.q_lo < 0 || r.q_hi > 15)) return -1;
    if (r.Cin != e.Cout || r.Cout != e.Cin || r.N != e.N || r.H != e.H || r.W != e.W || e.Cout % 128) return -1;
    int k = 0;
    for (int i = 0; i < NUM_E2; ++i)
        if (kE2[i].c == e.Cin && ++k == nth) return i;
    return -1;
}

}

int er2_num_variants(const hawq_expand_reduce_args *a) {
    int n = 0;
    while (e2_variant(a, n + 1) >= 0) ++n;
    return n;
}

int er2_launch(const hawq_expand_reduce_args *a, int nth, void *stream) {
    const int v = e2_variant(a, nth);
    HAWQ_REQUIRE(v >= 0, "hawq_conv_expand_reduce: no pipelined variant %d for this launch", nth);
    const hawq_conv_args &e = a->expand, &r = a->reduce;
    auto e_fast = [](int ek) { return (ek & 0xff) >= 33 && (ek & 0xff) <= 62; };
    HAWQ_REQUIRE(e.mq >= 0 && e_fast(e.eq) && e.m_id_scalar >= 0 && e_fast(e.e_id_scalar), "hawq_conv_expand_reduce: scalar tables outside the fast contract");
    HAWQ_REQUIRE(e.q_lo <= 0, "hawq_conv_expand_reduce: the block-input QuantAct clamp must admit 0");
    HAWQ_REQUIRE(e.q_hi >= 0 && e.q_hi <= 32767, "hawq_conv_expand_reduce: q_hi outside [0, 32767]");
    E2P p;
    p.x2 = (const uint8_t *)e.in, p.w3 = (const uint8_t *)e.wgt, p.w1 = (const uint8_t *)r.wgt;
    p.ctab3 = e.ctab, p.ctab1 = r.ctab;
    p.res_in = (const uint16_t *)e.res_in, p.res_out = (uint16_t *)e.res_out;
    p.y = (uint8_t *)r.out_q;
    const long long M = (long long)e.N * e.H * e.W;
    HAWQ_REQUIRE(M > 0 && M < (1ll << 30), "hawq_conv_expand_reduce: bad problem size");
    p.M = (int)M, p.C3 = e.Cout;
    p.m_id_s = e.m_id_scalar, p.e_id_s = e.e_id_scalar, p.mq = e.mq, p.eq = e.eq, p.q_hi = e.q_hi;
    p.y_lo = r.relu && r.q_lo < 0 ? 0 : r.q_lo, p.y_hi = r.q_hi;
    p.y_planar = r.out_planar;
    p.y_nib = r.out_bits == 4;
    p.flags = e.flags;
    p.dbgbuf = nullptr;
    p.dbg = 0;
#ifdef HAWQ_ABLATE
    static const int dbg_env = HAWQ_DBG_ENV();
    p.dbg = dbg_env;
    static long long *dbg_dev = nullptr;
    if ((dbg_env & 128) && !dbg_dev) (void)hipMalloc(&dbg_dev, 16 * sizeof(long long));
    if (dbg_env & 128) p.dbgbuf = dbg_dev;
#endif
    const E2Info &ei = kE2[v];
    static const bool attrs = [] {
        bool good = true;
        for (const E2Info &k : kE2)
            for (int i = 0; i < 5; ++i)
                good &= hipFuncSetAttribute((const void *)k.fn[i], hipFuncAttributeMaxDynamicSharedMemorySize, k.lds) == hipSuccess;
        return good;
    }();
    HAWQ_REQUIRE(attrs, "hawq_conv_expand_reduce: hipFuncSetAttribute(MaxDynamicSharedMemorySize) failed");
    const bool tie = ((e.fast_tables | r.fast_tables) & 4) != 0, ck0 = (e.fast_tables & 8) && (r.fast_tables & 8);
    const bool qk0 = (e.eq >> 8) == 0 && ids0_form(e.e_id_scalar);
    hipLaunchKernelGGL(ei.fn[tie ? 1 : (ck0 ? (qk0 ? 3 : 2) : (qk0 ? 4 : 0))], dim3((p.M + ei.bm - 1) / ei.bm), dim3(ei.nt), ei.lds, (hipStream_t)stream, p);
    HAWQ_CHECK_HIP(hipGetLastError());
    if (p.dbgbuf) {
        long long hb[12];
        (void)hipStreamSynchronize((hipStream_t)stream);
        (void)hipMemcpy(hb, p.dbgbuf, sizeof(hb), hipMemcpyDeviceToHost);
        fprintf(stderr, "[pipelined C=%d bm=%d M=%d C3=%d] cycles of compute wave 0 / workgroup 8: prologue + iteration 0 %lld | barrier wait %lld | stores %lld | GEMM1 %lld | "
                        "epilogue 1 + GEMM2 %lld | tail %lld || producer wave 0: prologue %lld | barrier wait %lld | issue %lld | vmcnt wait %lld\n",
                ei.c, ei.bm, p.M, p.C3, hb[0], hb[1], hb[2], hb[3], hb[4], hb[5], hb[8], hb[9], hb[10], hb[11]);
    }
    return 0;
}
```

### hawq_amd/csrc/fused_wp.hip

```cpp
#include <stdio.h>
#include <utility>

#include "common.h"

namespace {

struct WPP {
    const uint8_t *x2, *w3, *w1;
    const int32_t *ctab3, *ctab1;
    const uint16_t *res_in;
    uint16_t *res_out;
    uint8_t *y;
    uint8_t *q_out;
    int q_nib;
    int M, C3;
    int m_id_s, e_id_s, mq, eq, q_hi;
    int y_lo, y_hi, y_planar, y_nib;
    int spb;
    int32_t *flags;
    long long *dbgbuf;
};

template <int... Is, class Fn>
__device__ __forceinline__ void sfor_impl(std::integer_sequence<int, Is...>, Fn &&f) {
    (f(std::integral_constant<int, Is>{}), ...);
}
template <int N, class Fn>
__device__ __forceinline__ void sfor(Fn &&f) {
    sfor_impl(std::make_integer_sequence<int, N>{}, f);
}

__device__ __forceinline__ void wp_dma16(const char *src, char *dst) {
    __builtin_amdgcn_global_load_lds((const __attribute__((address_space(1))) void *)src, (__attribute__((address_space(3))) void *)dst, 16, 0, 0);
}
__device__ __forceinline__ void wp_dma4(const char *src, char *dst) {
    __builtin_amdgcn_global_load_lds((const __attribute__((address_space(1))) void *)src, (__attribute__((address_space(3))) void *)dst, 4, 0, 0);
}
template <bool K0>
__device__ __forceinline__ DyNt wp_ctab(const char *ctab, int ch) {
    const v4i t = *reinterpret_cast<const v4i *>(ctab + ch * 16);
    DyNt d;
    d.m = t.x, d.s = K0 ? t.y : (t.y & 31), d.k = K0 ? 0 : (t.y >> 8);
    d.add = (long long)(((unsigned long long)(unsigned)t.w << 32) | (unsigned)t.z);
    return d;
}

template <int C_, int NW_, bool REDUCE_, int MINW_>
struct WPCfg {
    static constexpr int C = C_, NW = NW_, MINW = MINW_;
    static constexpr bool REDUCE = REDUCE_;
    static constexpr int NT = 64 * NW, BM = 32 * NW;
    static constexpr int KC = C / 64;
    static constexpr int CT2 = C / 32;
    static constexpr int RPP = NT / 4;
    static constexpr int W3_BYTES = 64 * C;
    static constexpr int W1_BYTES = REDUCE ? 64 * C : 0;
    static constexpr int STAGE = W3_BYTES + W1_BYTES;
    static constexpr int W3PASS = (64 * KC + RPP - 1) / RPP, W1PASS = REDUCE ? (C + RPP - 1) / RPP : 0;
    static constexpr int CTPASS = NW >= 4 ? 1 : 4 / NW;
    static constexpr int NDMA = W3PASS + W1PASS + CTPASS;
    static constexpr int OFF_CT = 2 * STAGE;
    static constexpr int OFF_STG = OFF_CT + 2 * 1024;
    static constexpr int LDS_BYTES = OFF_STG + NW * 4096;
    static_assert(RPP % 16 == 0 && (NW == 1 || NW == 2 || NW % 4 == 0), "producer passes must cover whole swizzle groups");
};

template <class F, bool TIE, bool CK0, bool QK0 = false>
__global__ __launch_bounds__(F::NT, F::MINW) void expand_wp_kernel(const WPP p) {
    extern __shared__ __attribute__((aligned(16))) char smem[];
    constexpr int MODE_S = TIE ? 2 : 0;
    constexpr int MODE_Q = TIE ? 2 : (QK0 ? 1 : 0);
    constexpr int MODE_C = TIE ? 2 : (CK0 ? 1 : 0);
    constexpr bool K0 = CK0 && !TIE;
    constexpr int C = F::C;
    const int t = threadIdx.x, lane = t & 63, wave = t >> 6, l31 = lane & 31, h = lane >> 5;
    const int pix = blockIdx.x * F::BM + wave * 32 + l31;
    const bool valid = pix < p.M;
    const size_t row = valid ? pix : p.M - 1;
    const int nsl = p.C3 >> 6;
    const int j0 = blockIdx.y * p.spb, j1 = (j0 + p.spb < nsl) ? j0 + p.spb : nsl;
    char *ct = smem + F::OFF_CT;
    const int prow = t >> 2, pslot = t & 3;
    const int sw = (pslot ^ ((prow >> 2) & 3)) << 4;
    auto issue = [&](int j, int stage) {
        char *dst = smem + stage * F::STAGE;
#pragma unroll
        for (int i = 0; i < F::W3PASS; ++i) {
            const int idx = (i * F::RPP + prow) & (64 * F::KC - 1), first = (i * F::RPP + wave * 16) & (64 * F::KC - 1);
            wp_dma16((const char *)p.w3 + (size_t)(j * 64 + (idx & 63)) * C + (idx >> 6) * 64 + sw, dst + first * 64);
        }
#pragma unroll
        for (int i = 0; i < F::W1PASS; ++i) {
            const int r = (i * F::RPP + prow) & (C - 1), first = (i * F::RPP + wave * 16) & (C - 1);
            wp_dma16((const char *)p.w1 + (size_t)r * p.C3 + j * 64 + sw, dst + F::W3_BYTES + first * 64);
        }
#pragma unroll
        for (int i = 0; i < F::CTPASS; ++i) {
            const int q4 = (wave + i * F::NW) & 3;
            wp_dma4((const char *)p.ctab3 + (size_t)j * 1024 + q4 * 256 + lane * 4, ct + (j & 1) * 1024 + q4 * 256);
        }
    };
    char *stg = smem + F::OFF_STG + wave * 4096;
    const int pix0 = blockIdx.x * F::BM + wave * 32;
    const int crow = lane >> 3, cslot = lane & 7;
    unsigned coff[4];
#pragma unroll
    for (int k = 0; k < 4; ++k) {
        const int r = 8 * k + crow;
        coff[k] = (unsigned)((pix0 + r < p.M) ? pix0 + r : p.M - 1) * (unsigned)(p.C3 * 2) + ((cslot ^ (r & 7)) << 4);
    }
    auto dma_res = [&](int j) {
#pragma unroll
        for (int k = 0; k < 4; ++k) wp_dma16((const char *)p.res_in + (coff[k] + (unsigned)(j * 128)), stg + k * 1024);
    };
    const unsigned sl = lds_addr(stg) + l31 * 128;
    const int x7 = l31 & 7;
    v4i xf[F::KC][2];
    {
        const int r2 = lane >> 2, s2 = lane & 3;
#pragma unroll
        for (int kc0 = 0; kc0 < F::KC; kc0 += 2) {
#pragma unroll
            for (int kc = kc0; kc < kc0 + 2 && kc < F::KC; ++kc)
#pragma unroll
                for (int k = 0; k < 2; ++k) {
                    const int r = 16 * k + r2;
                    const size_t gr = (pix0 + r < p.M) ? pix0 + r : p.M - 1;
                    wp_dma16((const char *)p.x2 + gr * C + kc * 64 + ((s2 ^ ((r >> 2) & 3)) << 4), stg + (kc - kc0) * 2048 + k * 1024);
                }
            wait_vmcnt<0>();
#pragma unroll
            for (int kc = kc0; kc < kc0 + 2 && kc < F::KC; ++kc)
#pragma unroll
                for (int ks = 0; ks < 2; ++ks)
                    xf[kc][ks] = *reinterpret_cast<const v4i *>(stg + (kc - kc0) * 2048 + lds_off(l31, 2 * ks + h));
            asm volatile("s_waitcnt lgkmcnt(0)" ::: "memory");
#pragma unroll
            for (int kc = kc0; kc < kc0 + 2 && kc < F::KC; ++kc) pin(xf[kc][0]), pin(xf[kc][1]);
        }
    }
    issue(j0, 0);
    dma_res(j0);
    v16i acc2[F::REDUCE ? F::CT2 : 1];
    if constexpr (F::REDUCE) {
#pragma unroll
        for (int c = 0; c < F::CT2; ++c)
#pragma unroll
            for (int r = 0; r < 16; ++r) acc2[c][r] = 0;
    }
    DyNt dids = dynt_prepare(p.m_id_s, p.e_id_s), dq = dynt_prepare(p.mq, p.eq);
    constexpr bool SC0 = QK0 && !TIE;
    DyS0 dis0 = dys0_prepare(p.m_id_s, p.e_id_s);
    asm volatile("" : "+s"(dids.add), "+s"(dq.add), "+s"(dis0.add));
    const unsigned rowmask = valid ? 0xffffffffu : 0u;
    const int qhi2 = (p.q_hi & 0xffff) | (p.q_hi << 16);
    unsigned oor = 0;
    const int cp = cperm(l31);
    const unsigned a0 = lds_addr(smem) + lds_off(cp, h), a1 = lds_addr(smem) + lds_off(cp, 2 + h);
#ifdef HAWQ_ABLATE
    const bool prof = p.dbgbuf != nullptr;
    long long ph[8] = {0, 0, 0, 0, 0, 0, 0, 0};
    long long tprev = prof ? (long long)__builtin_readcyclecounter() : 0;
#define WP_STAMP(K)                                                    \
    if (prof) {                                                        \
        const long long now = (long long)__builtin_readcyclecounter(); \
        ph[K] += now - tprev;                                          \
        tprev = now;                                                   \
    }
#else
#define WP_STAMP(K)
#endif
    for (int j = j0; j < j1; ++j) {
        const int st = (j - j0) & 1;
        wait_vmcnt<4>();
        __builtin_amdgcn_s_barrier();
        WP_STAMP(0)
        const bool more = j + 1 < j1;
        if (more) issue(j + 1, st ^ 1);
        WP_STAMP(1)
        v16i acc1[2];
#pragma unroll
        for (int r = 0; r < 16; ++r) acc1[0][r] = 0, acc1[1][r] = 0;
        {
            const unsigned b0 = a0 + st * F::STAGE, b1 = a1 + st * F::STAGE;
            v4i wf[2][2];
            wf[0][0] = lds_read16<0>(b0), wf[0][1] = lds_read16<2048>(b0);
            sfor<2 * F::KC>([&](auto SI) {
                constexpr int s = decltype(SI)::value, kc = s >> 1, ks = s & 1, cur = s & 1, nxt = cur ^ 1;
                if constexpr (s + 1 < 2 * F::KC) {
                    constexpr int kn = (s + 1) >> 1;
                    wf[nxt][0] = lds_read16<kn * 4096>(ks ? b0 : b1), wf[nxt][1] = lds_read16<kn * 4096 + 2048>(ks ? b0 : b1);
                    wait_lgkm<2>();
                } else {
                    wait_lgkm<0>();
                }
                pin(wf[cur][0]), pin(wf[cur][1]);
                acc1[0] = __builtin_amdgcn_mfma_i32_32x32x32_i8(wf[cur][0], xf[kc][ks], acc1[0], 0, 0, 0);
                acc1[1] = __builtin_amdgcn_mfma_i32_32x32x32_i8(wf[cur][1], xf[kc][ks], acc1[1], 0, 0, 0);
            });
        }
        WP_STAMP(2)
        if (more) wait_vmcnt<F::NDMA>(); else wait_vmcnt<0>();
        v4i rin[4];
        rin[0] = lds_read16<0>(sl + ((4 * 0 + 2 * h) ^ x7) * 16), rin[1] = lds_read16<0>(sl + ((4 * 0 + 2 * h + 1) ^ x7) * 16);
        rin[2] = lds_read16<0>(sl + ((4 * 1 + 2 * h) ^ x7) * 16), rin[3] = lds_read16<0>(sl + ((4 * 1 + 2 * h + 1) ^ x7) * 16);
        wait_lgkm<0>();
        pin(rin[0]), pin(rin[1]), pin(rin[2]), pin(rin[3]);
        WP_STAMP(3)
        v4i qf[2];
        v4i rout[4];
// ... 60 lines not shown
                }
            }
        }
        asm volatile("s_waitcnt lgkmcnt(0)" ::: "memory");
        if (more) dma_res(j + 1);
        WP_STAMP(5)
        if constexpr (F::REDUCE) {
            const unsigned b0 = a0 + st * F::STAGE + F::W3_BYTES, b1 = a1 + st * F::STAGE + F::W3_BYTES;
            v4i wf[2][2];
            wf[0][0] = lds_read16<0>(b0), wf[0][1] = lds_read16<0>(b1);
            sfor<F::CT2>([&](auto CI) {
                constexpr int c = decltype(CI)::value, cur = c & 1, nxt = cur ^ 1;
                if constexpr (c + 1 < F::CT2) {
                    wf[nxt][0] = lds_read16<(c + 1) * 2048>(b0), wf[nxt][1] = lds_read16<(c + 1) * 2048>(b1);
                    wait_lgkm<2>();
                } else {
                    wait_lgkm<0>();
                }
                pin(wf[cur][0]), pin(wf[cur][1]);
                acc2[c] = __builtin_amdgcn_mfma_i32_32x32x32_i8(wf[cur][0], qf[0], acc2[c], 0, 0, 0);
                acc2[c] = __builtin_amdgcn_mfma_i32_32x32x32_i8(wf[cur][1], qf[1], acc2[c], 0, 0, 0);
            });
        }
        WP_STAMP(6)
    }
#ifdef HAWQ_ABLATE
    if (prof && blockIdx.x == 8 && blockIdx.y == 0 && t == 0)
        for (int k = 0; k < 8; ++k) p.dbgbuf[k] = ph[k];
#endif
#undef WP_STAMP
    if ((oor >> 16) != 0) atomicOr(p.flags, 1);
    if constexpr (F::REDUCE) {
        wait_vmcnt<0>();
#pragma unroll
        for (int c = 0; c < F::CT2; ++c) {
            const int ch0 = 32 * c + 16 * h;
            int w[4];
#pragma unroll
            for (int g = 0; g < 4; ++g) {
                int qv[4];
#pragma unroll
                for (int k = 0; k < 4; ++k)
                    qv[k] = med3i(dyadic_mode<MODE_C>(acc2[c][4 * g + k], wp_ctab<K0>((const char *)p.ctab1, ch0 + 4 * g + k)), p.y_lo, p.y_hi);
                w[g] = pack4_fast(qv[0], qv[1], qv[2], qv[3]);
            }
            const v4i ww = {w[0], w[1], w[2], w[3]};
            if (valid && p.y_nib) {
                const v2i nn = {w[0] | (w[1] << 4), w[2] | (w[3] << 4)};
                if (p.y_planar)
                    *reinterpret_cast<v2i *>((char *)p.y + ((size_t)(ch0 >> 5) * p.M + row) * 16 + ((ch0 >> 4) & 1) * 8) = nn;
                else
                    *reinterpret_cast<v2i *>((char *)p.y + row * (C / 2) + (ch0 >> 1)) = nn;
            } else if (valid) {
                if (p.y_planar)
                    *reinterpret_cast<v4i *>((char *)p.y + ((size_t)(ch0 >> 4) * p.M + row) * 16) = ww;
                else
                    *reinterpret_cast<v4i *>((char *)p.y + row * C + ch0) = ww;
            }
        }
    }
}

typedef void (*WPFn)(const WPP);
struct WPInfo { WPFn fn[5]; int c, bm, nt, lds; bool reduce; int ysplit; };
#define WP_ENTRY(F, YS) {{expand_wp_kernel<F, false, false>, expand_wp_kernel<F, false, true>, expand_wp_kernel<F, true, false>, expand_wp_kernel<F, false, true, true>, \
                          expand_wp_kernel<F, false, false, true>}, F::C, F::BM, F::NT, F::LDS_BYTES, F::REDUCE, YS}
using W64 = WPCfg<64, 4, true, 3>;
using W64B = WPCfg<64, 8, true, 3>;
using W128 = WPCfg<128, 4, true, 2>;
using W128B = WPCfg<128, 8, true, 2>;
using W256 = WPCfg<256, 4, true, 1>;
using N64 = WPCfg<64, 4, false, 4>;
using N128 = WPCfg<128, 4, false, 3>;
using N256 = WPCfg<256, 4, false, 3>;
using N512 = WPCfg<512, 4, false, 2>;
const WPInfo kWP[] = {WP_ENTRY(W64, 1), WP_ENTRY(W64B, 1), WP_ENTRY(W128, 1), WP_ENTRY(W128B, 1), WP_ENTRY(W256, 1),
                      WP_ENTRY(N64, 1), WP_ENTRY(N128, 1), WP_ENTRY(N256, 1), WP_ENTRY(N256, 2), WP_ENTRY(N256, 4),
                      WP_ENTRY(N512, 1), WP_ENTRY(N512, 2), WP_ENTRY(N512, 4), WP_ENTRY(N512, 8)};
constexpr int NUM_WP = sizeof(kWP) / sizeof(kWP[0]);

bool wp_expand_ok(const hawq_conv_args &e) {
    return (e.in_pitch == 0 || e.in_pitch == e.Cin) && (e.out_pitch == 0 || e.out_pitch == e.Cout) && e.KH == 1 && e.KW == 1 && e.stride == 1 && e.pad == 0 && e.in_bits == 8 && e.w_bits == 8 && e.fast_tables != 0 && !e.in2 &&
           !e.in_planar && e.epilogue == HAWQ_EPI_RESIDUAL && e.res_in && e.res_in_bits == 16 && (!e.res_out || e.res_out_bits == 16) &&
           e.flags && e.ctab && e.Cout % 64 == 0 && (e.out_bits == 8 || (e.out_bits == 4 && e.q_lo >= 0 && e.q_hi <= 15));
}

int wp_variant(const hawq_expand_reduce_args *a, int nth) {
    const hawq_conv_args &e = a->expand, &r = a->reduce;
    if (!wp_expand_ok(e)) return -1;
    const bool reduce = r.wgt != nullptr;
    if (reduce && e.out_bits != 8) return -1;
    if (reduce) {
        if (!(r.KH == 1 && r.KW == 1 && r.stride == 1 && r.pad == 0 && r.in_bits == 8 && r.w_bits == 8 && r.fast_tables != 0 && !r.in2)) return -1;
        if (r.epilogue != HAWQ_EPI_REQUANT || !r.ctab || !r.out_q || (r.out_bits != 8 && r.out_bits != 4) || !e.res_out) return -1;
        if (r.out_bits == 4 && (r.q_lo < 0 || r.q_hi > 15)) return -1;
        if (r.Cin != e.Cout || r.Cout != e.Cin || r.N != e.N || r.H != e.H || r.W != e.W) return -1;
    }
    int n = 0;
    for (int i = 0; i < NUM_WP; ++i)
        if (kWP[i].c == e.Cin && kWP[i].reduce == reduce && (e.Cout / 64) % kWP[i].ysplit == 0 && ++n == nth) return i;
    return -1;
}

}

int wp_num_variants(const hawq_expand_reduce_args *a) {
    int n = 0;
    while (wp_variant(a, n + 1) >= 0) ++n;
    return n;
}

int wp_launch(const hawq_expand_reduce_args *a, int nth, void *stream) {
    const int v = wp_variant(a, nth);
    HAWQ_REQUIRE(v >= 0, "hawq_conv_expand_reduce: no wave-private variant %d for this launch", nth);
    const hawq_conv_args &e = a->expand, &r = a->reduce;
    auto e_fast = [](int ek) { return (ek & 0xff) >= 33 && (ek & 0xff) <= 62; };
    HAWQ_REQUIRE(e.mq >= 0 && e_fast(e.eq) && e.m_id_scalar >= 0 && e_fast(e.e_id_scalar), "hawq_conv_expand_reduce: scalar tables outside the fast contract");
    HAWQ_REQUIRE(e.q_lo <= 0, "hawq_conv_expand_reduce: the block-input QuantAct clamp must admit 0");
    const WPInfo &wi = kWP[v];
    WPP p;
    p.x2 = (const uint8_t *)e.in, p.w3 = (const uint8_t *)e.wgt, p.w1 = (const uint8_t *)r.wgt;
    p.ctab3 = e.ctab, p.ctab1 = wi.reduce ? r.ctab : nullptr;
    p.res_in = (const uint16_t *)e.res_in, p.res_out = (uint16_t *)e.res_out;
    p.y = wi.reduce ? (uint8_t *)r.out_q : nullptr;
    p.q_out = wi.reduce ? nullptr : (uint8_t *)e.out_q;
    p.q_nib = !wi.reduce && e.out_bits == 4;
    const long long M = (long long)e.N * e.H * e.W;
    HAWQ_REQUIRE(M > 0 && M * e.Cout * 2 < (1ll << 32), "hawq_conv_expand_reduce: bad problem size");
    p.M = (int)M, p.C3 = e.Cout;
    p.m_id_s = e.m_id_scalar, p.e_id_s = e.e_id_scalar, p.mq = e.mq, p.eq = e.eq, p.q_hi = e.q_hi;
    p.y_lo = wi.reduce ? (r.relu && r.q_lo < 0 ? 0 : r.q_lo) : 0, p.y_hi = wi.reduce ? r.q_hi : 0;
    p.y_planar = wi.reduce ? r.out_planar : 0;
    p.y_nib = wi.reduce && r.out_bits == 4;
    p.spb = (e.Cout / 64) / wi.ysplit;
    p.flags = e.flags;
    p.dbgbuf = nullptr;
#ifdef HAWQ_ABLATE
    static const int dbg_env = HAWQ_DBG_ENV();
    static long long *dbg_dev = nullptr;
    if ((dbg_env & 128) && !dbg_dev) (void)hipMalloc(&dbg_dev, 8 * sizeof(long long));
    if (dbg_env & 128) p.dbgbuf = dbg_dev;
#endif
    static const bool attrs = [] {
        bool good = true;
        for (const WPInfo &k : kWP)
            for (int i = 0; i < 5; ++i)
                good &= hipFuncSetAttribute((const void *)k.fn[i], hipFuncAttributeMaxDynamicSharedMemorySize, k.lds) == hipSuccess;
        return good;
    }();
    HAWQ_REQUIRE(attrs, "hawq_conv_expand_reduce: hipFuncSetAttribute(MaxDynamicSharedMemorySize) failed");
    const int ft = e.fast_tables | (wi.reduce ? r.fast_tables : 0);
    const bool tie = (ft & 4) != 0, ck0 = (e.fast_tables & 8) && (!wi.reduce || (r.fast_tables & 8));
    const bool qk0 = (e.eq >> 8) == 0 && ids0_form(e.e_id_scalar);
    HAWQ_REQUIRE(e.q_hi >= 0 && e.q_hi <= 32767, "hawq_conv_expand_reduce: q_hi outside [0, 32767]");
    hipLaunchKernelGGL(wi.fn[tie ? 2 : (ck0 ? (qk0 ? 3 : 1) : (qk0 ? 4 : 0))], dim3((p.M + wi.bm - 1) / wi.bm, wi.ysplit), dim3(wi.nt), wi.lds, (hipStream_t)stream, p);
    HAWQ_CHECK_HIP(hipGetLastError());
    if (p.dbgbuf) {
        long long hb[8];
        (void)hipStreamSynchronize((hipStream_t)stream);
        (void)hipMemcpy(hb, p.dbgbuf, sizeof(hb), hipMemcpyDeviceToHost);
        fprintf(stderr, "[wave-private C=%d bm=%d reduce=%d ysplit=%d M=%d C3=%d] cycles of wave 0 / workgroup 8 over %d slices: wait+barrier %lld | issue ring DMA %lld | "
                        "GEMM1 %lld | wait + read residual %lld | epilogue %lld | stage + store + residual DMA %lld | GEMM2 %lld\n",
                wi.c, wi.bm, (int)wi.reduce, wi.ysplit, p.M, p.C3, p.spb, hb[0], hb[1], hb[2], hb[3], hb[4], hb[5], hb[6]);
    }
    return 0;
}
```

### hawq_amd/csrc/gemm_v2.hip

```cpp
#include <stdio.h>
#include <stdlib.h>

#include <type_traits>

#include "common.h"

namespace {

struct G2P {
    const char *x, *w;
    const char *x2, *w2;
    const int32_t *ctab, *ctab_id;
    const int32_t *bias;
    int32_t *out_acc;
    char *out;
    const char *res_in;
    char *res_out;
    int *flags;
    int M, K, Cout, n1, n2;
    int Ho, Wo, H1, W1, s1, H2, W2, K2, s2;
    int out_planar, out_bits, q_lo, q_hi;
    int mq, eq, m_id, e_id;
    unsigned x_bytes, w_bytes, x2_bytes, w2_bytes;
    int dbg;
// ... 335 lines not shown
                    }
                    if (m0 + wm * 64 + q * 32 + l31 < p.M) oor |= (unsigned)(o[0] | o[1]) | (unsigned)(o[2] | o[3]);
                    rp[2 * gq] = pack2_u16_sat(o[0], o[1]);
                    rp[2 * gq + 1] = pack2_u16_sat(o[2], o[3]);
                    w[gq] = pack4_min(qv[0], qv[1], qv[2], qv[3], qhi2);
                }
            }
            const int m = m0 + wm * 64 + q * 32 + l31;
            if (m < p.M && !HAWQ_DBG_BIT(p.dbg, 8)) {
                if (EPI == HAWQ_EPI_RESIDUAL && p.res_out) {
                    v4i *dst = reinterpret_cast<v4i *>(p.res_out + ((size_t)m * p.Cout + c0 + lch) * 2);
                    const v4i ra = {rp[0], rp[1], rp[2], rp[3]}, rb = {rp[4], rp[5], rp[6], rp[7]};
                    dst[0] = ra, dst[1] = rb;
                }
                if (p.out && p.out_bits == 8) {
                    const v4i ww = {w[0], w[1], w[2], w[3]};
                    char *dst = p.out_planar ? p.out + ((size_t)((c0 + lch) >> 4) * p.M + m) * 16 : p.out + (size_t)m * p.Cout + c0 + lch;
                    *reinterpret_cast<v4i *>(dst) = ww;
                } else if (p.out) {
                    const int ch = c0 + lch;
                    const v2i ww = {w[0] | (w[1] << 4), w[2] | (w[3] << 4)};
                    char *dst = p.out_planar ? p.out + ((size_t)(ch >> 5) * p.M + m) * 16 + ((ch >> 4) & 1) * 8 : p.out + (((size_t)m * p.Cout + ch) >> 1);
                    *reinterpret_cast<v2i *>(dst) = ww;
                }
            }
        }
    }
    if (EPI == HAWQ_EPI_RESIDUAL && (oor >> 16) != 0 && p.res_out && !HAWQ_DBG_BIT(p.dbg, ~0)) atomicOr(p.flags, 1);
    if (prof && blockIdx.x == 8 && t == 0) {
        p.dbgbuf[0] = t_begin - t_entry, p.dbgbuf[1] = t_loop_end - t_begin;
        p.dbgbuf[2] = (long long)__builtin_readcyclecounter() - t_loop_end, p.dbgbuf[3] = total;
        p.dbgbuf[4] = t_b0 - t_begin;
    }
}

using G64D = G2Cfg<1, 5, 2>;
using G64S = G2Cfg<1, 3, 2>;
using G128 = G2Cfg<2, 4, 2>;
constexpr int NUM_G2 = 3;

typedef void (*G2Fn)(const G2P);
struct G2Info { G2Fn fn[2][3][2]; G2Fn raw[2]; int bn, lds, nt; };
#define G2_FNS(CFG, N) {{gemm1x1_v2_kernel<CFG, HAWQ_EPI_REQUANT, false, 0, N>, gemm1x1_v2_kernel<CFG, HAWQ_EPI_REQUANT, false, 2, N>},    \
                        {gemm1x1_v2_kernel<CFG, HAWQ_EPI_RESIDUAL, false, 0, N>, gemm1x1_v2_kernel<CFG, HAWQ_EPI_RESIDUAL, false, 2, N>},  \
                        {gemm1x1_v2_kernel<CFG, HAWQ_EPI_RESIDUAL, true, 0, N>, gemm1x1_v2_kernel<CFG, HAWQ_EPI_RESIDUAL, true, 2, N>}}
#define G2_ENTRY(CFG) {{G2_FNS(CFG, false), G2_FNS(CFG, true)}, {gemm1x1_v2_kernel<CFG, HAWQ_EPI_RAW, false, 0, false>, gemm1x1_v2_kernel<CFG, HAWQ_EPI_RAW, false, 0, true>}, \
                       CFG::BN, CFG::LDS_BYTES, CFG::NT}
const G2Info kG2[NUM_G2] = {G2_ENTRY(G64D), G2_ENTRY(G64S), G2_ENTRY(G128)};

}

int gemm_v2_count(void) { return NUM_G2; }

extern "C" int hawq_pack_w1x1_k128(const int8_t *src, int8_t *dst, int32_t N, int32_t K) {
    HAWQ_REQUIRE(src && dst && N > 0 && K > 0 && N % 64 == 0 && K % 128 == 0, "hawq_pack_w1x1_k128: N must be a positive multiple of 64, K of 128");
    const int nch = K >> 7;
    for (int g = 0; g < (N >> 6); ++g)
        for (int ch = 0; ch < nch; ++ch) {
            int8_t *tile = dst + ((size_t)g * nch + ch) * 8192;
            for (int r = 0; r < 64; ++r) {
                const int8_t *row = src + (size_t)(g * 64 + r) * K + ch * 128;
                for (int sl = 0; sl < 8; ++sl)
                    for (int b = 0; b < 16; ++b) tile[r * 128 + ((sl ^ ((r >> 1) & 7)) << 4) + b] = row[sl * 16 + b];
            }
        }
    return 0;
}

bool gemm_v2_applies(const hawq_conv_args *a, int v) {
    if (v < 0 || v >= NUM_G2) return false;
    const G2Info &gi = kG2[v];
    const bool dual = a->in2 != nullptr;
    const bool nib = a->in_bits == 4 && a->w_bits == 4;
    const int rowb = nib ? a->Cin >> 1 : a->Cin, rowb2 = nib ? a->Cin2 >> 1 : a->Cin2;
    const long long Ho = (a->H - 1) / a->stride + 1, Wo = (a->W - 1) / a->stride + 1, M = (long long)a->N * Ho * Wo, Min = (long long)a->N * a->H * a->W;
    const bool qout_ok = a->out_bits == 8 || (a->out_bits == 4 && a->q_lo >= 0 && a->q_hi <= 15 && a->Cout % 32 == 0);
    const bool raw = a->epilogue == HAWQ_EPI_RAW;
    const bool epi_ok = (raw && a->out_acc && a->bias && !dual) ||
                        (a->epilogue == HAWQ_EPI_REQUANT && a->out_q && qout_ok && (a->out_bits == 8 || a->relu || a->q_lo >= 0) && !dual) ||
                        (a->epilogue == HAWQ_EPI_RESIDUAL && (dual || (a->res_in && a->res_in_bits == 16)) && (!a->res_out || (a->res_out_bits == 16 && a->flags)) &&
                         !a->res_no_relu && !a->res_clamp16 && (a->res_out || a->out_q) && (!a->out_q || qout_ok));
    const bool dual_ok = !dual || (a->wgt2_k128 && a->ctab_id && a->in2_bits == a->in_bits && a->w2_bits == a->w_bits && rowb2 % 128 == 0 &&
                                   (long long)a->N * a->H2 * a->W2 * rowb2 < (1ll << 31) && (long long)a->Cout * rowb2 < (1ll << 31));
    return a->KH == 1 && a->KW == 1 && a->stride >= 1 && a->pad == 0 && (raw || (a->fast_tables != 0 && a->ctab)) && a->wgt_k128 != nullptr && !a->in_planar && epi_ok && dual_ok &&
           ((a->in_bits == 8 && a->w_bits == 8) || nib) && rowb % 128 == 0 && a->Cout % gi.bn == 0 && (a->in_pitch == 0 || a->in_pitch == rowb) &&
           (a->out_pitch == 0 || a->out_pitch == a->Cout) && Min * rowb < (1ll << 31) && (long long)a->Cout * rowb < (1ll << 31) && M * a->Cout < (1ll << 31);
}

int gemm_v2_launch(const hawq_conv_args *a, int v, int exact_tie, int dbg, void *stream) {
    const G2Info &gi = kG2[v];
    const bool dual = a->in2 != nullptr;
    const bool nib = a->in_bits == 4;
    const int rowb = nib ? a->Cin >> 1 : a->Cin, rowb2 = nib ? a->Cin2 >> 1 : a->Cin2;
    G2P p;
    p.x = (const char *)a->in, p.w = (const char *)a->wgt_k128, p.x2 = (const char *)a->in2, p.w2 = (const char *)a->wgt2_k128;
    p.ctab = a->ctab, p.ctab_id = a->ctab_id;
    p.bias = a->bias, p.out_acc = a->out_acc;
    p.out = (char *)a->out_q, p.res_in = (const char *)a->res_in, p.res_out = (char *)a->res_out, p.flags = a->flags;
    p.Ho = (a->H - 1) / a->stride + 1, p.Wo = (a->W - 1) / a->stride + 1, p.M = a->N * p.Ho * p.Wo, p.K = rowb, p.Cout = a->Cout;
    p.H1 = a->H, p.W1 = a->W, p.s1 = a->stride;
    p.n1 = rowb >> 7, p.n2 = dual ? rowb2 >> 7 : 0;
    p.H2 = a->H2, p.W2 = a->W2, p.K2 = rowb2, p.s2 = a->stride2;
    p.out_planar = a->out_planar, p.out_bits = a->out_bits;
    p.q_lo = a->relu && a->q_lo < 0 ? 0 : a->q_lo, p.q_hi = a->q_hi;
    p.mq = a->mq, p.eq = a->eq, p.m_id = a->m_id_scalar, p.e_id = a->e_id_scalar;
    if (a->epilogue != HAWQ_EPI_RESIDUAL || !a->out_q) p.mq = 0, p.eq = 33;
    if (a->epilogue != HAWQ_EPI_RESIDUAL || dual) p.m_id = 0, p.e_id = 33;
    p.x_bytes = (unsigned)((long long)a->N * a->H * a->W * rowb), p.w_bytes = (unsigned)((long long)a->Cout * rowb);
    p.x2_bytes = dual ? (unsigned)((long long)a->N * a->H2 * a->W2 * rowb2) : 0, p.w2_bytes = dual ? (unsigned)((long long)a->Cout * rowb2) : 0;
    p.dbg = dbg;
    static long long *dbg_dev = nullptr;
    if (HAWQ_DBG_BIT(dbg, 128) && !dbg_dev) (void)hipMalloc(&dbg_dev, 8 * sizeof(long long));
    p.dbgbuf = HAWQ_DBG_BIT(dbg, 128) ? dbg_dev : nullptr;
    static const bool attrs = [] {
        bool good = true;
        for (const G2Info &i : kG2) {
            for (int k = 0; k < 12; ++k) good &= hipFuncSetAttribute((const void *)i.fn[k / 6][(k % 6) >> 1][k & 1], hipFuncAttributeMaxDynamicSharedMemorySize, i.lds) == hipSuccess;
            for (int k = 0; k < 2; ++k) good &= hipFuncSetAttribute((const void *)i.raw[k], hipFuncAttributeMaxDynamicSharedMemorySize, i.lds) == hipSuccess;
        }
        return good;
    }();
    HAWQ_REQUIRE(attrs, "hawq_conv2d: hipFuncSetAttribute failed for the round-5 1x1 kernels");
    const int grid = ((p.M + 127) / 128) * (p.Cout / gi.bn);
    const int e = a->epilogue == HAWQ_EPI_REQUANT ? 0 : (dual ? 2 : 1);
    G2Fn fn = a->epilogue == HAWQ_EPI_RAW ? gi.raw[nib ? 1 : 0] : gi.fn[nib ? 1 : 0][e][exact_tie ? 1 : 0];
    hipLaunchKernelGGL(fn, dim3(grid), dim3(gi.nt), gi.lds, (hipStream_t)stream, p);
    HAWQ_CHECK_HIP(hipGetLastError());
    if (p.dbgbuf) {
        long long hb[5];
        (void)hipStreamSynchronize((hipStream_t)stream);
        (void)hipMemcpy(hb, p.dbgbuf, sizeof(hb), hipMemcpyDeviceToHost);
        fprintf(stderr, "[gemm-v2 %d bn=%d M=%d K=%d(+%d) Cout=%d grid=%d lds=%d] chunks %lld: prologue %lld | K loop %lld | epilogue %lld cycles (wave 0 of workgroup 8); first operands %lld\n",
                v, gi.bn, p.M, a->Cin, dual ? a->Cin2 : 0, p.Cout, grid, gi.lds, hb[3], hb[0], hb[1], hb[2], hb[4]);
    }
    return 0;
}
```

### hawq_amd/engine.py

```python
from __future__ import annotations

import ctypes as C
import os
import sys
from functools import partial

import numpy as np
import torch

from . import _lib, packing
from .quant_utils import requant_table, tables_are_fast, tables_fit_fast
from .runner import EventTimer, GraphRunner, _act_range, _i32, two_round_min


RES_VBITS = 20
U16_VBITS = 17


def _no_preshift(ek) -> bool:
    return bool((np.asarray(ek, dtype=np.int64) >> 8 == 0).all())


class _OpList(list):

    def __init__(self):
        super().__init__()
        self.names = []
        self.next_name = None

    def append(self, fn):
        name = self.next_name or (fn.args[0] if hasattr(fn, "args") else "op")
        self.names.append(name)
        self.next_name = None
        super().append(fn)


class StalePlan(ValueError):
    """A recorded plan does not fit the launch list / kernel inventory of this build: the engine falls back to tuning."""


SPLITK_CANDIDATES = (2, 4, 8, 16, 32)


class _SplitWorkspace:

    def __init__(self, dev):
        self.dev, self.slab, self.counters = dev, None, None

    def fit(self, a, slices):
        slab, cnt = C.c_int64(), C.c_int64()
        _lib.call("hawq_conv2d_splitk_workspace", C.byref(a), slices, C.byref(slab), C.byref(cnt))
        if self.slab is None or self.slab.numel() < slab.value:
            self.slab = torch.zeros(slab.value, dtype=torch.uint8, device=self.dev)
        if self.counters is None or self.counters.numel() < cnt.value // 4:
            self.counters = torch.zeros(cnt.value // 4, dtype=torch.int32, device=self.dev)

    def launch(self, a, slices, stream):
        if slices:
            _lib.call("hawq_conv2d_splitk", C.byref(a), slices, self.slab.data_ptr(), self.counters.data_ptr(), stream)
        else:
            _lib.call("hawq_conv2d", C.byref(a), stream)


class _ConvLaunch:

    def __init__(self, a, ws, stream):
        self.a, self.ws, self.sp, self.splitk = a, ws, stream, 0

    def __call__(self):
        self.ws.launch(self.a, self.splitk, self.sp)


class _FusedPair:

    def __init__(self, er, expand, reduce, stream, ws):
        self.er, self.expand, self.reduce, self.sp = er, expand, reduce, stream
        self.fused = True
        self.ws, self.split_e, self.split_r = ws, 0, 0

    def __call__(self):
        if self.fused:
            _lib.call("hawq_conv_expand_reduce", C.byref(self.er), self.sp)
        else:
            self.ws.launch(self.expand, self.split_e, self.sp)
            if self.reduce is not None:
                self.ws.launch(self.reduce, self.split_r, self.sp)


class _Conv:

    def __init__(self, mod, s_a, in_bits, dev, from_buffers, in_range=None):
        if not from_buffers:
            mod.prepare(s_a)
        w_int = mod.weight_integer.detach().cpu().numpy()
        self.cout, self.cin, self.kh, self.kw = w_int.shape
        self.stride, self.pad = int(mod.conv.stride[0]), int(mod.conv.padding[0])
        if mod.conv.groups != 1 or mod.conv.dilation[0] != 1:
            raise NotImplementedError("grouped/dilated convolutions are outside the ResNet hot path")
        self.w_bits = 4 if (mod.weight_bit <= 4 and in_bits == 4) else 8
# ... 508 lines not shown
        self._lut_key = None

    def _time_graph(self, reps: int = 8) -> float:
        ms = super()._time_graph(reps)
        self.flags.zero_()
        return ms

    def _build_chains(self, N, H, W, x_view=None, logits_view=None):
        P, dev = self.P, self.dev
        self._drop_graph()
        if self.chains > 1 and N >= 2 * self.chains:
            self.x_in = torch.empty(N, 3, H, W, dtype=torch.float32, device=dev)
            self.logits = torch.empty(N, P['fc']['nout'], dtype=torch.float32, device=dev)
            self.subs, b0 = [], 0
            split = [int(v) for v in os.environ.get("HAWQ_SPLIT", "").split(",") if v]
            if len(split) != self.chains or sum(split) != N or min(split) < 1:
                split = [N // self.chains + (1 if i < N % self.chains else 0) for i in range(self.chains)]
            for i in range(self.chains):
                b1 = b0 + split[i]
                sub = IntegerEngine(None, _parent=self)
                sub._chain_index = i
                sub._plan_on = getattr(self, "_plan_on", False)
                sub._build(b1 - b0, H, W, self.x_in[b0:b1], self.logits[b0:b1])
                self.subs.append(sub)
                b0 = b1
            self._ops, self._keep, self._batch, self._graph = _OpList(), [], (N, H, W), None
            if (self.autotune and not self._fixed("tiles") and os.environ.get("HAWQ_JOINT_TUNE", "1") != "0"
                    and all(hasattr(sub, "_tile_times") for sub in self.subs)):
                self._autotune_joint()
            self.n_fast, self.n_conv, self.n_k0, self.n_tie = (self.subs[0].n_fast, self.subs[0].n_conv, self.subs[0].n_k0,
                                                              self.subs[0].n_tie)
            self.n_ck0 = self.subs[0].n_ck0
            self.tile_choice, self.er_choice = self.subs[0].tile_choice, self.subs[0].er_choice
            self.er_split_tiles = getattr(self.subs[0], "er_split_tiles", {})
            return
        self.subs = []
        ops, keep = _OpList(), []
        self._conv_args, self._conv_names = [], []
        self._conv_ops = []
        self._ws = _SplitWorkspace(dev)
        self.acc_taps = {}
        self.res_taps = {}
        self.n_fast = self.n_conv = self.n_k0 = self.n_tie = self.n_ck0 = 0
        sp = self.stream.cuda_stream
        ptr = lambda t: None if t is None else t.data_ptr()
        rdt = torch.uint16 if self.res_bits == 16 else torch.int32
        self.x_in = x_view if x_view is not None else torch.empty(N, 3, H, W, dtype=torch.float32, device=dev)
        Ho, Wo = (H + 6 - 7) // 2 + 1, (W + 6 - 7) // 2 + 1
        Hp, Wp = 2 * (Ho - 1) + 7 + 1, 2 * (Wo - 1) + 8
        Hp, Wp = max(Hp, H + 3), max(Wp + (Wp & 1), W + 3 + ((W + 3) & 1))
        unfused = self.keep_acc or bool(os.environ.get("HAWQ_UNFUSED_STEM"))
        xq = torch.zeros(N * Hp * Wp * 4, dtype=torch.int8, device=dev) if unfused else None
        st = P['stem']
        stem16 = self._alloc(N * Ho * Wo * 64, torch.uint16) if unfused else None
        stem_acc = self._alloc(N * Ho * Wo * 64, torch.int32) if self.keep_acc else None
        if stem_acc is not None:
            self.acc_taps['stem'] = (stem_acc, (N, Ho, Wo, 64))
        H1, W1 = (Ho + 2 - 3) // 2 + 1, (Wo + 2 - 3) // 2 + 1
        units = P['units']
        u0 = units[0]
        res = self._alloc(N * H1 * W1 * 64, torch.uint16) if not u0['resize'] else None
        qa = self._alloc(N * H1 * W1 * 64 * u0['a_bits'] // 8, torch.uint8)
        c = st['conv']
        if self.keep_acc or os.environ.get("HAWQ_UNFUSED_STEM"):
            ops.append(partial(_lib.call, "hawq_quantize_input", self.x_in.data_ptr(), xq.data_ptr(), N, 3, H, W, Hp, Wp,
                               3, 3, P['inv_s_in'], -128, 127, sp))
            ops.append(partial(_lib.call, "hawq_stem_conv7", xq.data_ptr(), c.w.data_ptr(), c.bias.data_ptr(),
                               st['m'].data_ptr(), st['e'].data_ptr(), N, Hp, Wp, Ho, Wo, st['rng'][0], st['rng'][1],
                               stem16.data_ptr(), ptr(stem_acc), sp))
            ops.append(partial(_lib.call, "hawq_maxpool3s2_requant", stem16.data_ptr(), N, Ho, Wo, 64, ptr(res),
                               qa.data_ptr(), u0['a_bits'], u0['mq'], u0['eq'], u0['a_rng'][0], u0['a_rng'][1], sp))
        else:
            ops.append(partial(_lib.call, "hawq_stem_fused", self.x_in.data_ptr(), N, 3, H, W, P['inv_s_in'], -128, 127,
                               c.w.data_ptr(), c.bias.data_ptr(), st['m'].data_ptr(), st['e'].data_ptr(), st['rng'][0],
                               st['rng'][1], ptr(res), qa.data_ptr(), u0['a_bits'], u0['mq'], u0['eq'], u0['a_rng'][0],
                               u0['a_rng'][1], int(st['fast'] and self.fast), sp))
            self._stem_u8_tail = (c.w.data_ptr(), c.bias.data_ptr(), st['m'].data_ptr(), st['e'].data_ptr(), st['rng'][0],
                                  st['rng'][1], ptr(res), qa.data_ptr(), u0['a_bits'], u0['mq'], u0['eq'], u0['a_rng'][0],
                                  u0['a_rng'][1], int(st['fast'] and self.fast), sp)
        keep += [xq, stem16, stem_acc, res, qa]
        h, w = H1, W1
        res_bits_in = 16
        fused_in = None
        self._er_args, self._er_names = [], []
        for ui, u in enumerate(units):
            nxt = units[ui + 1] if ui + 1 < len(units) else None
            x_in, x_bits, hin, win, x_planar = qa, u['a_bits'], h, w, False
            for ci, ent in enumerate(u['convs']):
                c = ent['conv']
                if ci == 0 and fused_in is not None:
                    x_in, x_bits, x_planar = fused_in
                    hin, win = (hin + 2 * c.pad - c.kh) // c.stride + 1, (win + 2 * c.pad - c.kw) // c.stride + 1
                    fused_in = None
                    self.n_fast += 1
                    self.n_conv += 1
                    continue
                ho, wo = (hin + 2 * c.pad - c.kh) // c.stride + 1, (win + 2 * c.pad - c.kw) // c.stride + 1
                a = _lib.ConvArgs()
                a.in_, a.wgt, a.bias = x_in.data_ptr(), c.w.data_ptr(), c.bias.data_ptr()
                if x_bits == c.w_bits and c.band() is not None:
                    a.wgt_band = c.band().data_ptr()
                if x_bits == c.w_bits and c.k128() is not None:
                    a.wgt_k128 = c.k128().data_ptr()
                a.N, a.H, a.W, a.Cin, a.Cout = N, hin, win, c.cin, c.cout
                a.KH, a.KW, a.stride, a.pad = c.kh, c.kw, c.stride, c.pad
                a.in_bits, a.w_bits = x_bits, c.w_bits
                a.m, a.e = ent['m'].data_ptr(), ent['e'].data_ptr()
                a.flags = self.flags.data_ptr()
                a.fast_tables = int(bool(ent.get('fast', False)) and self.res_bits == 16 and self.fast)
                if a.fast_tables and ent.get('tie', False):
                    a.fast_tables = 5
                elif a.fast_tables and ent.get('k0', False):
                    a.fast_tables = 3
                self.n_tie += int(a.fast_tables == 5)
                self.n_k0 += int(a.fast_tables == 3)
                if a.fast_tables and ent.get('ck0', False):
                    a.fast_tables |= 8
                    self.n_ck0 += 1
                if a.fast_tables:
                    a.ctab = ent['ctab'].data_ptr()
                    if ci == len(u['convs']) - 1 and u['resize']:
                        a.ctab_id = u['ctab_id'].data_ptr()
                self.n_fast += int(a.fast_tables != 0)
                self.n_conv += 1
                a.tile = int(os.environ.get("HAWQ_TILE_RES" if ci == len(u['convs']) - 1 else "HAWQ_TILE_REQ", "0"))
                a.in_planar = int(x_planar)
                tap_name = f"{u['name']}.quant_convbn{ci + 1}"
                if ci < len(u['convs']) - 1:
                    out = self._alloc(N * ho * wo * c.cout * ent['out_bits'] // 8, torch.uint8)
                    a.epilogue, a.relu = _lib.EPI_REQUANT, 1
                    a.out_q, a.out_bits, a.q_lo, a.q_hi = out.data_ptr(), ent['out_bits'], ent['rng'][0], ent['rng'][1]
                    keep.append(out)
                    x_next, xb_next = out, ent['out_bits']
                    planar_next = bool(a.fast_tables) and self.planar and self._band_takes(u['convs'][ci + 1], N, ho, wo, xb_next,
                                                                                            ci + 1 == len(u['convs']) - 1, u)
                    a.out_planar = int(planar_next)
                else:
                    a.epilogue = _lib.EPI_RESIDUAL
                    if u['resize']:
                        ic = u['ident']
                        a.in2, a.wgt2, a.bias2 = qa.data_ptr(), ic.w.data_ptr(), ic.bias.data_ptr()
                        if u['a_bits'] == ic.w_bits and ic.k128() is not None:
                            a.wgt2_k128 = ic.k128().data_ptr()
                        a.H2, a.W2, a.Cin2, a.stride2 = h, w, ic.cin, ic.stride
                        a.in2_bits, a.w2_bits = u['a_bits'], ic.w_bits
                        a.m_id, a.e_id = u['m_id'].data_ptr(), u['e_id'].data_ptr()
                    else:
                        a.res_in, a.res_in_bits = res.data_ptr(), res_bits_in
                        a.m_id_scalar, a.e_id_scalar = u['m_id_s'], u['e_id_s']
                    need_res = (nxt is None) or (not nxt['resize'])
                    new_res = self._alloc(N * ho * wo * c.cout, rdt) if need_res else None
                    if new_res is not None:
                        a.res_out, a.res_out_bits = new_res.data_ptr(), self.res_bits
                        self.res_taps[u['name']] = (new_res, (N, ho, wo, c.cout))
                    new_qa = None
                    if nxt is not None:
                        a.out_bits = nxt['a_bits']
                        a.q_lo, a.q_hi, a.mq, a.eq = nxt['a_rng'][0], nxt['a_rng'][1], nxt['mq'], nxt['eq']
                    keep.append(new_res)
                if self.keep_acc:
                    self._add_acc_tap(ops, keep, a, tap_name, N, ho, wo, c.cout)
                    if ci == len(u['convs']) - 1 and u['resize']:
                        self._add_ident_tap(ops, keep, u, qa, N, h, w, ho, wo)
                keep.append(a)
                fz = self._try_fuse(a, u, nxt, N, ho, wo, keep) if (ci == len(u['convs']) - 1 and not self.keep_acc) else None
                if fz is None and ci == len(u['convs']) - 1 and nxt is not None:
                    new_qa = self._alloc(N * ho * wo * c.cout * nxt['a_bits'] // 8, torch.uint8)
                    a.out_q = new_qa.data_ptr()
                    keep.append(new_qa)
                if fz is not None:
                    pair, fout, fbits, fplanar = fz
                    fused_in = (fout, fbits, fplanar)
                    self._er_args.append(pair)
                    self._er_names.append(tap_name)
                    ops.next_name = tap_name + "+" + nxt['name'] + ".quant_convbn1"
                    ops.append(pair)
                    continue
                solo = self._try_solo(a, u, keep) if (ci == len(u['convs']) - 1 and not self.keep_acc) else None
                if solo is not None:
                    self._er_args.append(solo)
                    self._er_names.append(tap_name + "@solo")
                    ops.next_name = tap_name
                    ops.append(solo)
                    continue
                self._conv_args.append(a)
                self._conv_names.append(tap_name)
                self._conv_ops.append(_ConvLaunch(a, self._ws, sp))
                ops.next_name = tap_name + ("+identity" if (a.in2 is not None) else "")
                ops.append(self._conv_ops[-1])
                if ci < len(u['convs']) - 1:
                    x_in, x_bits, hin, win, x_planar = x_next, xb_next, ho, wo, planar_next
            res, qa, h, w = new_res, new_qa, ho, wo
            res_bits_in = self.res_bits
        cl = units[-1]['convs'][-1]['conv'].cout
        qf = self._alloc(N * cl, torch.int8)
        pooled = self._alloc(N * cl, torch.int32) if self.keep_acc else None
        if pooled is not None:
            self.acc_taps['final_pool'] = (pooled, (N, cl))
        o = P['out']
        ops.append(partial(_lib.call, "hawq_avgpool_requant", res.data_ptr(), self.res_bits, N, h * w, cl, qf.data_ptr(),
                           ptr(pooled), o['mq'], o['eq'], o['rng'][0], o['rng'][1], sp))
        fc = P['fc']
        if fc['k'] != cl:
            raise RuntimeError("FC input width does not match the last stage")
        self.logits = logits_view if logits_view is not None else torch.empty(N, fc['nout'], dtype=torch.float32, device=dev)
        a = _lib.ConvArgs()
        a.in_, a.wgt, a.bias = qf.data_ptr(), fc['w'].data_ptr(), fc['bias'].data_ptr()
        a.N, a.H, a.W, a.Cin, a.Cout, a.KH, a.KW, a.stride, a.pad = N, 1, 1, fc['k'], fc['nout_p'], 1, 1, 1, 0
        a.in_bits, a.w_bits = 8, 8
        a.epilogue = _lib.EPI_DEQUANT
        a.out_f32, a.fscale, a.ldo, a.n_valid = self.logits.data_ptr(), fc['fscale'].data_ptr(), fc['nout'], fc['nout']
        if self.keep_acc:
            self._add_acc_tap(ops, keep, a, 'quant_output', N, 1, 1, fc['nout_p'])
        ops.next_name = "quant_output"
        if _lib.load().hawq_fc_dequant_ok(N, fc['k'], fc['nout_p']) and not os.environ.get("HAWQ_NO_FC2"):
            ops.append(partial(_lib.call, "hawq_fc_dequant", qf.data_ptr(), fc['w'].data_ptr(), fc['bias'].data_ptr(), fc['fscale'].data_ptr(),
                               self.logits.data_ptr(), N, fc['k'], fc['nout_p'], fc['nout'], fc['nout'], sp))
        else:
            self._conv_ops.append(_ConvLaunch(a, self._ws, sp))
            ops.append(self._conv_ops[-1])
            self._conv_args.append(a)
            self._conv_names.append("quant_output")
        keep += [qf, pooled, a]
        self._ops, self._keep, self._batch = ops, keep, (N, H, W)
        self._graph = None
        if self.autotune and not self.keep_acc:
            self._autotune_tiles()

    def _add_acc_tap(self, ops, keep, a, name, N, ho, wo, cout):
        acc = self._alloc(N * ho * wo * cout, torch.int32)
        r = _lib.ConvArgs()
        C.memmove(C.byref(r), C.byref(a), C.sizeof(r))
        r.in2 = None
        r.epilogue, r.out_acc = _lib.EPI_RAW, acc.data_ptr()
        keep += [acc, r]
        self.acc_taps[name] = (acc, (N, ho, wo, cout))
        ops.append(partial(_lib.call, "hawq_conv2d", C.byref(r), self.stream.cuda_stream))

    def _add_ident_tap(self, ops, keep, u, qa, N, h, w, ho, wo):
        ic = u['ident']
        acc = self._alloc(N * ho * wo * ic.cout, torch.int32)
        r = _lib.ConvArgs()
        r.in_, r.wgt, r.bias = qa.data_ptr(), ic.w.data_ptr(), ic.bias.data_ptr()
        r.N, r.H, r.W, r.Cin, r.Cout, r.KH, r.KW, r.stride, r.pad = N, h, w, ic.cin, ic.cout, 1, 1, ic.stride, 0
        r.in_bits, r.w_bits = u['a_bits'], ic.w_bits
        r.epilogue, r.out_acc = _lib.EPI_RAW, acc.data_ptr()
        keep += [acc, r]
        self.acc_taps[u['name'] + ".quant_identity_convbn"] = (acc, (N, ho, wo, ic.cout))
        ops.append(partial(_lib.call, "hawq_conv2d", C.byref(r), self.stream.cuda_stream))

    def _autotune_tiles(self, reps: int = 3):
        n_tiles = _lib.load().hawq_conv2d_num_tiles()
        sp = self.stream.cuda_stream
        self._tile_times, self._er_times = {}, {}
        retired = {int(v) for v in os.environ.get("HAWQ_RETIRED_TILES", "5,19").split(",") if v}
        fixed = self._fixed("tiles")
        if fixed:
            ids = [int(v) for v in fixed.split(".")]
            names = (self.plan or {}).get("conv_launches") if getattr(self, "_plan_on", False) else None
            if names is not None and len(names) == len(ids) and list(names) != list(self._conv_names):
                if [n for n in names if n not in self._UNTUNED_SINCE] != list(self._conv_names):
                    raise StalePlan("recorded for another launch list (other network, schedule or storage rule)")
                by_name = dict(zip(names, ids))
                ids = [by_name[n] for n in self._conv_names]
            if len(ids) != len(self._conv_args):
                raise StalePlan(f"the recorded plan lists {len(ids)} tiles, this plan has {len(self._conv_args)} conv launches")
            counts = self.plan.get("pair_variant_counts") if getattr(self, "_plan_on", False) else None
            if counts is not None and list(counts) != [int(_lib.load().hawq_conv_expand_reduce_variants(C.byref(p.er))) for p in self._er_args]:
                raise StalePlan("the fused expand(-> reduce) kernels of this build are numbered differently")
            for name, a, tid in zip(self._conv_names, self._conv_args, ids):
                a.tile = tid
                self.tile_choice[name] = tid
            split = self._fixed("fused_split_tiles")
            split = [int(x) for x in split.split(".")] if split else None
            self.er_split_tiles = getattr(self, "er_split_tiles", {})
# ... 262 lines not shown
```

### include/hawq_mi355.h

```cpp
#ifndef HAWQ_MI355_H
#define HAWQ_MI355_H

#include <stdint.h>

#ifdef __cplusplus
extern "C" {
#endif

#define HAWQ_ABI_VERSION 5

const char *hawq_last_error(void);
int hawq_abi_version(void);
int hawq_device_ok(void);

enum {
    HAWQ_EPI_RAW = 0,
    HAWQ_EPI_REQUANT = 1,
    HAWQ_EPI_RESIDUAL = 2,
    HAWQ_EPI_DEQUANT = 3
};

typedef struct hawq_conv_args {
    const void *in;
    const void *wgt;
    const int32_t *bias;
    int32_t N, H, W, Cin, Cout, KH, KW, stride, pad;
    int32_t in_bits, w_bits;
    const void *in2;
    const void *wgt2;
    const int32_t *bias2;
    int32_t H2, W2, Cin2, stride2, in2_bits, w2_bits;
    int32_t epilogue;
    int32_t relu;
    const int32_t *m;
    const int32_t *e;
    const int32_t *m_id;
    const int32_t *e_id;
    int32_t m_id_scalar, e_id_scalar;
    const void *res_in;
    int32_t res_in_bits;
    void *res_out;
    int32_t res_out_bits;
    void *out_q;
    int32_t out_bits;
    int32_t q_lo, q_hi;
    int32_t mq, eq;
    int32_t *out_acc;
    float *out_f32;
    const float *fscale;
    int32_t ldo, n_valid;
    int32_t *flags;
    int32_t tile;
    const int32_t *ctab;
    const int32_t *ctab_id;
    int32_t fast_tables;
    int32_t in_planar;
    int32_t out_planar;
    int32_t res_no_relu, res_clamp16;
    int32_t in_pitch, out_pitch;
    const void *wgt_band;
    const void *wgt_k128;
    const void *wgt2_k128;
} hawq_conv_args;

int hawq_conv2d(const hawq_conv_args *args, void *stream);
int hawq_conv2d_num_tiles(void);
int hawq_conv2d_num_band_tiles(void);
int hawq_conv2d_band_tile(const hawq_conv_args *args);
int hawq_conv2d_num_band2_tiles(void);
int hawq_conv2d_band2_tile(const hawq_conv_args *args);
int hawq_pack_w3x3_band(const int8_t *src, int8_t *dst, int32_t Cout, int32_t Cin);
int hawq_conv2d_num_gemm2_tiles(void);
int hawq_conv2d_gemm2_first(void);
int hawq_pack_w1x1_k128(const int8_t *src, int8_t *dst, int32_t Cout, int32_t Cin);

int hawq_conv2d_splitk_ok(const hawq_conv_args *args, int32_t slices);
int hawq_conv2d_splitk_workspace(const hawq_conv_args *args, int32_t slices, int64_t *slab_bytes, int64_t *counter_bytes);
int hawq_conv2d_splitk(const hawq_conv_args *args, int32_t slices, void *slab, int32_t *counters, void *stream);

typedef struct hawq_expand_reduce_args {
    hawq_conv_args expand;
    hawq_conv_args reduce;
    int32_t tile;
} hawq_expand_reduce_args;
int hawq_conv_expand_reduce(const hawq_expand_reduce_args *args, void *stream);
int hawq_conv_expand_reduce_variants(const hawq_expand_reduce_args *args);

int hawq_quantize_input(const float *x, int8_t *out, int32_t N, int32_t C, int32_t H, int32_t W,
                        int32_t out_h, int32_t out_w, int32_t pad_top, int32_t pad_left,
                        float inv_scale, int32_t lo, int32_t hi, void *stream);

int hawq_stem_conv7(const int8_t *in, const int8_t *wgt, const int32_t *bias, const int32_t *m,
                    const int32_t *e, int32_t N, int32_t Hp, int32_t Wp, int32_t Ho, int32_t Wo,
                    int32_t q_lo, int32_t q_hi, uint16_t *out16, int32_t *out_acc, void *stream);

int hawq_stem_fused(const float *x, int32_t N, int32_t C, int32_t H, int32_t W, float inv_scale, int32_t in_lo,
                    int32_t in_hi, const int8_t *wgt, const int32_t *bias, const int32_t *m, const int32_t *e,
                    int32_t a_lo, int32_t a_hi, uint16_t *res_out, void *out_q, int32_t out_bits, int32_t mq,
                    int32_t eq, int32_t q_lo, int32_t q_hi, int32_t fast_tables, void *stream);

int hawq_stem_fused_u8(const uint8_t *x, const int8_t *lut, int32_t N, int32_t C, int32_t H, int32_t W,
                       const int8_t *wgt, const int32_t *bias, const int32_t *m, const int32_t *e, int32_t a_lo,
                       int32_t a_hi, uint16_t *res_out, void *out_q, int32_t out_bits, int32_t mq, int32_t eq,
                       int32_t q_lo, int32_t q_hi, int32_t fast_tables, void *stream);

int hawq_maxpool3s2_requant(const uint16_t *in, int32_t N, int32_t H, int32_t W, int32_t C,
                            uint16_t *res_out, void *out_q, int32_t out_bits, int32_t mq, int32_t eq,
                            int32_t q_lo, int32_t q_hi, void *stream);

int hawq_requant_residual(const void *in, int32_t in_bits, int64_t n, void *out_q, int32_t out_bits,
                          int32_t mq, int32_t eq, int32_t q_lo, int32_t q_hi, void *stream);

int hawq_avgpool_requant(const void *in, int32_t in_bits, int32_t N, int32_t HW, int32_t C, int8_t *out,
                         int32_t *pooled_out, int32_t mq, int32_t eq, int32_t q_lo, int32_t q_hi,
                         void *stream);

int hawq_fc_dequant_ok(int32_t N, int32_t K, int32_t Nout_p);
int hawq_fc_dequant(const int8_t *q, const int8_t *wgt, const int32_t *bias, const float *fscale, float *out_f32, int32_t N, int32_t K,
                    int32_t Nout_p, int32_t n_valid, int32_t ldo, void *stream);


int hawq_f32_nchw_to_q_nhwc(const float *x, void *out, int32_t N, int32_t C, int32_t H, int32_t W,
                            int32_t Cpad, int32_t bits, float scale, void *stream);
int hawq_acc_nhwc_to_f32_nchw(const int32_t *acc, float *y, int32_t N, int32_t C, int32_t H, int32_t W,
                              int32_t Cpad, const float *fscale, void *stream);
int hawq_fixedpoint_f32(const float *z, float *y, int32_t N, int32_t C, int32_t HW, float s_a,
                        const float *s_w, const int32_t *m, const int32_t *e, int32_t per_ch,
                        const float *ident, float s_ida, const float *s_idw, const int32_t *m_id,
                        const int32_t *e_id, int32_t per_ch_id, float s_out, int32_t do_clamp,
                        int32_t q_lo, int32_t q_hi, void *stream);
int hawq_fakequant_f32(const float *x, float *y, int64_t n, float inv_scale, float scale, int32_t lo,
                       int32_t hi, void *stream);
int hawq_avgpool_f32(const float *x, float *y, int32_t NC, int32_t HW, float scale, void *stream);

int hawq_conv2d_grouped(const int8_t *in, const int8_t *wgt, const int32_t *bias, int32_t N, int32_t H, int32_t W,
                        int32_t Cin, int32_t Cout, int32_t KH, int32_t KW, int32_t stride, int32_t pad, int32_t groups,
                        int32_t *out_acc, void *stream);

int hawq_depthwise3x3(const int8_t *in, const int8_t *wgt9c, const int32_t *bias, int32_t N, int32_t H, int32_t W, int32_t C,
                      int32_t stride, int32_t *out_acc, void *stream);

int hawq_depthwise3x3_requant(const int8_t *in, const int8_t *wgt9c, const int32_t *bias, const int32_t *m, const int32_t *e,
                              int32_t N, int32_t H, int32_t W, int32_t C, int32_t C_valid, int32_t stride, int32_t relu, int32_t q_lo,
                              int32_t q_hi, int8_t *out_q, int32_t *out_acc, void *stream);

// ... 93 lines not shown
```

Before: 101,400.

## Compute only subsampled outputs when next unit's readers are strided 1x1 convs

Adds an out_sub field so the last conv of a unit that feeds a downsampling unit computes and writes only the pixels the next unit's strided 1x1 conv and identity path will read. The next unit then runs those convs at stride 1 on the compacted activation. The residual input is read from the full-resolution buffer through remapped row indices in the generic epilogue and the fused wide-path kernel. This cuts GEMM work and output traffic for the pre-downsample block, but disables the band, gemm_v2, splitk and several fused kernels for those launches, which may push them onto slower generic paths.

```diff
diff --git a/hawq_amd/_lib.py b/hawq_amd/_lib.py
--- a/hawq_amd/_lib.py
+++ b/hawq_amd/_lib.py
@@ -30,6 +30,7 @@
         ("res_no_relu", i32), ("res_clamp16", i32),
         ("in_pitch", i32), ("out_pitch", i32),
         ("wgt_band", vp), ("wgt_k128", vp), ("wgt2_k128", vp),
+        ("out_sub", i32),
     ]
 
 
diff --git a/hawq_amd/csrc/conv_igemm.hip b/hawq_amd/csrc/conv_igemm.hip
--- a/hawq_amd/csrc/conv_igemm.hip
+++ b/hawq_amd/csrc/conv_igemm.hip
@@ -35,6 +35,7 @@
     int in_planar, out_planar;
     int gfast;
     int in_pitch, out_pitch;
+    int res_sub;
     int dbg;
     long long *dbgbuf;
 };
@@ -433,6 +434,14 @@
 
 __device__ __forceinline__ v4i ld4(const int32_t *p) { return *reinterpret_cast<const v4i *>(p); }
 
+__device__ __forceinline__ size_t res_row(const ConvP &p, int pix) {
+    if (p.res_sub > 1) {
+        const int hw = p.Ho * p.Wo, n = pix / hw, r = pix - n * hw, oy = r / p.Wo, ox = r - oy * p.Wo;
+        return ((size_t)n * p.H + (size_t)oy * p.res_sub) * p.W + (size_t)ox * p.res_sub;
+    }
+    return (size_t)pix;
+}
+
 
 template <class C, int EPI, bool DUAL>
 __device__ __forceinline__ void epilogue_generic(const ConvP &p, v16i (&acc)[C::CT][C::PT],
@@ -440,6 +449,12 @@
     const int lane = threadIdx.x & 63, wave = threadIdx.x >> 6;
     const int wave_m = wave % C::WM, wave_c = wave / C::WM;
     const int l31 = lane & 31, h = lane >> 5;
+    size_t rrow[C::PT];
+#pragma unroll
+    for (int q = 0; q < C::PT; ++q) {
+        const int pix = m0 + wave_m * (C::PT * 32) + q * 32 + l31;
+        rrow[q] = (EPI == HAWQ_EPI_RESIDUAL && !DUAL) ? res_row(p, pix < p.M ? pix : 0) : (size_t)pix;
+    }
 #pragma unroll
     for (int c = 0; c < C::CT; ++c) {
         const int ch = c0 + wave_c * (C::CT * 32) + c * 32 + h * 16;
@@ -450,6 +465,7 @@
             constexpr bool PITCHED = EPI == HAWQ_EPI_REQUANT || EPI == HAWQ_EPI_RESIDUAL;
             const int opitch = PITCHED ? p.out_pitch : p.Cout;
             const size_t elem = (size_t)pix * opitch + ch;
+            const size_t relem = rrow[q] * opitch + ch;
             bool ovf = false;
             int qw[4] = {0, 0, 0, 0};
 #pragma unroll
@@ -486,8 +502,8 @@
                         const int av = acc[c][q][4 * g + j];
                         int ov = tie ? dyadic_tie(av, dm) : dyadic_nt(av, dm);
                         if (p.res_in) {
-                            const int r = p.res_in_bits == 16 ? (int)((const uint16_t *)p.res_in)[elem + 4 * g + j]
-                                                              : ((const int32_t *)p.res_in)[elem + 4 * g + j];
+                            const int r = p.res_in_bits == 16 ? (int)((const uint16_t *)p.res_in)[relem + 4 * g + j]
+                                                              : ((const int32_t *)p.res_in)[relem + 4 * g + j];
                             ov += tie ? dyadic_tie(r, dids) : dyadic_nt(r, dids);
                         }
                         if (!p.res_no_relu) ov = max(ov, 0);
@@ -533,8 +549,8 @@
                         } else if (p.res_in) {
 #pragma unroll
                             for (int j = 0; j < 4; ++j) {
-                                const int r = p.res_in_bits == 16 ? (int)((const uint16_t *)p.res_in)[elem + 4 * g + j]
-                                                                  : ((const int32_t *)p.res_in)[elem + 4 * g + j];
+                                const int r = p.res_in_bits == 16 ? (int)((const uint16_t *)p.res_in)[relem + 4 * g + j]
+                                                                  : ((const int32_t *)p.res_in)[relem + 4 * g + j];
                                 idv[j] = dyadic_rne(r, p.m_id_s, p.e_id_s);
                             }
                         } else {
@@ -604,8 +620,8 @@
         if (base >= C::BM * S::RCPR) break;
         const int idx = base + lane;
         const int row = idx / S::RCPR, j = idx % S::RCPR;
-        const int grow = (m0 + row < p.M) ? m0 + row : m0;
-        const char *src = (const char *)p.res_in + ((size_t)grow * p.Cout + c0) * 2 + ((j ^ S::rsw(row)) << 4);
+        const size_t grow = res_row(p, (m0 + row < p.M) ? m0 + row : m0);
+        const char *src = (const char *)p.res_in + (grow * p.Cout + c0) * 2 + ((j ^ S::rsw(row)) << 4);
         __builtin_amdgcn_global_load_lds((const __attribute__((address_space(1))) void *)src,
                                          (__attribute__((address_space(3))) void *)(res_tile + base * 16), 16, 0, 0);
     }
@@ -1213,7 +1229,7 @@
     const bool epi_ok = (a->epilogue == HAWQ_EPI_REQUANT && a->out_q) ||
                         (res && a->res_in && a->res_in_bits == 16 && (!a->res_out || a->res_out_bits == 16));
     const bool dense = (a->in_pitch == 0 || a->in_pitch == a->Cin * a->in_bits / 8) && (a->out_pitch == 0 || a->out_pitch == a->Cout);
-    return a->KH == 3 && a->KW == 3 && a->stride == 1 && a->pad == 1 && a->in2 == nullptr && a->fast_tables != 0 && epi_ok && dense &&
+    return a->KH == 3 && a->KW == 3 && a->stride == 1 && a->pad == 1 && a->out_sub < 2 && a->in2 == nullptr && a->fast_tables != 0 && epi_ok && dense &&
            ((a->in_bits == 8 && a->w_bits == 8) || (nib && a->Cin % 128 == 0)) && a->Cout % bi.bn == 0 &&
            band_rows * (wo + 2) <= bi.band_px - 4 && (bi.bstages > 1 || (a->Cin >> (nib ? 7 : 6)) == 1);
 }
@@ -1336,17 +1352,22 @@
                  "hawq_conv2d: in_bits/w_bits must be 4 or 8 (got %d/%d)", a->in_bits, a->w_bits);
     HAWQ_REQUIRE(a->KH > 0 && a->KW > 0 && a->stride > 0 && a->pad >= 0 && a->N > 0 && a->H > 0 && a->W > 0,
                  "hawq_conv2d: bad geometry");
+    const int sub = a->out_sub >= 2 ? a->out_sub : 1;
+    HAWQ_REQUIRE(sub == 1 || (a->KH == 1 && a->KW == 1 && a->stride == 1 && a->pad == 0 && !a->in2 && !a->res_out && a->epilogue == HAWQ_EPI_RESIDUAL &&
+                              !a->in_planar && !a->out_planar && a->in_pitch == 0 && a->out_pitch == 0),
+                 "hawq_conv2d: out_sub=%d needs a 1x1 / stride 1 / pad 0 single-branch RESIDUAL launch without res_out, dense NHWC rows", a->out_sub);
     ConvP p;
     p.in = (const uint8_t *)a->in;
     p.wgt = (const uint8_t *)a->wgt;
     p.bias = a->bias;
     p.N = a->N, p.H = a->H, p.W = a->W, p.Cin = a->Cin, p.Cout = a->Cout;
-    p.KH = a->KH, p.KW = a->KW, p.stride = a->stride, p.pad = a->pad;
-    p.Ho = (a->H + 2 * a->pad - a->KH) / a->stride + 1;
-    p.Wo = (a->W + 2 * a->pad - a->KW) / a->stride + 1;
+    p.KH = a->KH, p.KW = a->KW, p.stride = a->stride * sub, p.pad = a->pad;
+    p.res_sub = sub > 1 ? sub : 0;
+    p.Ho = (a->H + 2 * a->pad - a->KH) / p.stride + 1;
+    p.Wo = (a->W + 2 * a->pad - a->KW) / p.stride + 1;
     HAWQ_REQUIRE(p.Ho > 0 && p.Wo > 0, "hawq_conv2d: empty output");
     const long long M = (long long)a->N * p.Ho * p.Wo;
-    HAWQ_REQUIRE(M * (long long)a->Cout < (1ll << 40) && M < (1ll << 30), "hawq_conv2d: problem too large");
+    HAWQ_REQUIRE(M * (long long)a->Cout < (1ll << 40) && M < (1ll << 30) && (long long)a->N * a->H * a->W < (1ll << 30), "hawq_conv2d: problem too large");
     p.M = (int)M;
     p.in_bits = a->in_bits, p.w_bits = a->w_bits;
     const bool dual = a->in2 != nullptr;
diff --git a/hawq_amd/csrc/conv_splitk.hip b/hawq_amd/csrc/conv_splitk.hip
--- a/hawq_amd/csrc/conv_splitk.hip
+++ b/hawq_amd/csrc/conv_splitk.hip
@@ -109,6 +109,7 @@
     HAWQ_REQUIRE((k1 || k3) && (a->stride == 1 || a->stride == 2), "hawq_conv2d_splitk: 1x1 / pad 0 or 3x3 / pad 1 convs with stride 1 or 2 only");
     HAWQ_REQUIRE(a->n_valid == 0 && (a->in_pitch == 0 || a->in_pitch == a->Cin) && (a->out_pitch == 0 || a->out_pitch == a->Cout),
                  "hawq_conv2d_splitk: n_valid / in_pitch / out_pitch are not supported");
+    HAWQ_REQUIRE(a->out_sub < 2, "hawq_conv2d_splitk: out_sub is not supported");
     const int epi = a->epilogue;
     HAWQ_REQUIRE(epi == HAWQ_EPI_RAW || epi == HAWQ_EPI_REQUANT || epi == HAWQ_EPI_RESIDUAL, "hawq_conv2d_splitk: RAW, REQUANT or RESIDUAL epilogue only");
     HAWQ_REQUIRE(epi == HAWQ_EPI_RAW || !a->out_q || a->out_bits == 8, "hawq_conv2d_splitk: out_bits must be 8");
diff --git a/hawq_amd/csrc/fused_er.hip b/hawq_amd/csrc/fused_er.hip
--- a/hawq_amd/csrc/fused_er.hip
+++ b/hawq_amd/csrc/fused_er.hip
@@ -404,7 +404,7 @@
 
 int er_variant(const hawq_expand_reduce_args *a) {
     const hawq_conv_args &e = a->expand, &r = a->reduce;
-    if (!conv_is_1x1_int8_fast(e, true) || !conv_is_1x1_int8_fast(r)) return -1;
+    if (!conv_is_1x1_int8_fast(e, true) || !conv_is_1x1_int8_fast(r) || e.out_sub >= 2 || r.out_sub >= 2) return -1;
     const bool dual = e.in2 != nullptr;
     if (dual && !dual_branch_fits(e)) return -1;
     if (e.epilogue != HAWQ_EPI_RESIDUAL || r.epilogue != HAWQ_EPI_REQUANT) return -1;
diff --git a/hawq_amd/csrc/fused_er2.hip b/hawq_amd/csrc/fused_er2.hip
--- a/hawq_amd/csrc/fused_er2.hip
+++ b/hawq_amd/csrc/fused_er2.hip
@@ -366,7 +366,7 @@
 
 int e2_variant(const hawq_expand_reduce_args *a, int nth) {
     const hawq_conv_args &e = a->expand, &r = a->reduce;
-    if (!r.wgt || !e2_conv_ok(e) || !e2_conv_ok(r)) return -1;
+    if (!r.wgt || !e2_conv_ok(e) || !e2_conv_ok(r) || e.out_sub >= 2 || r.out_sub >= 2) return -1;
     if (e.epilogue != HAWQ_EPI_RESIDUAL || r.epilogue != HAWQ_EPI_REQUANT) return -1;
     if (!e.res_in || e.res_in_bits != 16 || !e.res_out || e.res_out_bits != 16 || !e.flags || !e.ctab || !r.ctab || !r.out_q) return -1;
     if ((r.out_bits != 8 && r.out_bits != 4) || e.out_bits != 8) return -1;
diff --git a/hawq_amd/csrc/fused_wp.hip b/hawq_amd/csrc/fused_wp.hip
--- a/hawq_amd/csrc/fused_wp.hip
+++ b/hawq_amd/csrc/fused_wp.hip
@@ -17,6 +17,7 @@
     int m_id_s, e_id_s, mq, eq, q_hi;
     int y_lo, y_hi, y_planar, y_nib;
     int spb;
+    int sub, sW, sHW, dW, dHW;
     int32_t *flags;
     long long *dbgbuf;
 };
@@ -80,6 +81,23 @@
     const int nsl = p.C3 >> 6;
     const int j0 = blockIdx.y * p.spb, j1 = (j0 + p.spb < nsl) ? j0 + p.spb : nsl;
     char *ct = smem + F::OFF_CT;
+    const int pix0 = blockIdx.x * F::BM + wave * 32;
+    auto srow = [&](int d) -> unsigned {
+        d = d < p.M ? d : p.M - 1;
+        if constexpr (!F::REDUCE) {
+            if (p.sub > 1) {
+                const int n = d / p.dHW, r = d - n * p.dHW, y = r / p.dW, x = r - y * p.dW;
+                return (unsigned)(n * p.sHW + (y * p.sW + x) * p.sub);
+            }
+        }
+        return (unsigned)d;
+    };
+    unsigned rsrc[4], xsrc[2];
+#pragma unroll
+    for (int k = 0; k < 4; ++k) rsrc[k] = srow(pix0 + 8 * k + (lane >> 3));
+#pragma unroll
+    for (int k = 0; k < 2; ++k) xsrc[k] = srow(pix0 + 16 * k + (lane >> 2));
+    asm volatile("" : "+v"(rsrc[0]), "+v"(rsrc[1]), "+v"(rsrc[2]), "+v"(rsrc[3]), "+v"(xsrc[0]), "+v"(xsrc[1]));
     const int prow = t >> 2, pslot = t & 3;
     const int sw = (pslot ^ ((prow >> 2) & 3)) << 4;
     auto issue = [&](int j, int stage) {
@@ -101,13 +119,12 @@
         }
     };
     char *stg = smem + F::OFF_STG + wave * 4096;
-    const int pix0 = blockIdx.x * F::BM + wave * 32;
     const int crow = lane >> 3, cslot = lane & 7;
     unsigned coff[4];
 #pragma unroll
     for (int k = 0; k < 4; ++k) {
         const int r = 8 * k + crow;
-        coff[k] = (unsigned)((pix0 + r < p.M) ? pix0 + r : p.M - 1) * (unsigned)(p.C3 * 2) + ((cslot ^ (r & 7)) << 4);
+        coff[k] = rsrc[k] * (unsigned)(p.C3 * 2) + ((cslot ^ (r & 7)) << 4);
     }
     auto dma_res = [&](int j) {
 #pragma unroll
@@ -125,7 +142,7 @@
 #pragma unroll
                 for (int k = 0; k < 2; ++k) {
                     const int r = 16 * k + r2;
-                    const size_t gr = (pix0 + r < p.M) ? pix0 + r : p.M - 1;
+                    const size_t gr = xsrc[k];
                     wp_dma16((const char *)p.x2 + gr * C + kc * 64 + ((s2 ^ ((r >> 2) & 3)) << 4), stg + (kc - kc0) * 2048 + k * 1024);
                 }
             wait_vmcnt<0>();
@@ -352,7 +369,8 @@
 bool wp_expand_ok(const hawq_conv_args &e) {
     return (e.in_pitch == 0 || e.in_pitch == e.Cin) && (e.out_pitch == 0 || e.out_pitch == e.Cout) && e.KH == 1 && e.KW == 1 && e.stride == 1 && e.pad == 0 && e.in_bits == 8 && e.w_bits == 8 && e.fast_tables != 0 && !e.in2 &&
            !e.in_planar && e.epilogue == HAWQ_EPI_RESIDUAL && e.res_in && e.res_in_bits == 16 && (!e.res_out || e.res_out_bits == 16) &&
-           e.flags && e.ctab && e.Cout % 64 == 0 && (e.out_bits == 8 || (e.out_bits == 4 && e.q_lo >= 0 && e.q_hi <= 15));
+           e.flags && e.ctab && e.Cout % 64 == 0 && (e.out_bits == 8 || (e.out_bits == 4 && e.q_lo >= 0 && e.q_hi <= 15)) &&
+           (e.out_sub < 2 || !e.res_out);
 }
 
 int wp_variant(const hawq_expand_reduce_args *a, int nth) {
@@ -360,6 +378,7 @@
     if (!wp_expand_ok(e)) return -1;
     const bool reduce = r.wgt != nullptr;
     if (reduce && e.out_bits != 8) return -1;
+    if (reduce && (e.out_sub >= 2 || r.out_sub >= 2)) return -1;
     if (reduce) {
         if (!(r.KH == 1 && r.KW == 1 && r.stride == 1 && r.pad == 0 && r.in_bits == 8 && r.w_bits == 8 && r.fast_tables != 0 && !r.in2)) return -1;
         if (r.epilogue != HAWQ_EPI_REQUANT || !r.ctab || !r.out_q || (r.out_bits != 8 && r.out_bits != 4) || !e.res_out) return -1;
@@ -395,9 +414,11 @@
     p.y = wi.reduce ? (uint8_t *)r.out_q : nullptr;
     p.q_out = wi.reduce ? nullptr : (uint8_t *)e.out_q;
     p.q_nib = !wi.reduce && e.out_bits == 4;
-    const long long M = (long long)e.N * e.H * e.W;
-    HAWQ_REQUIRE(M > 0 && M * e.Cout * 2 < (1ll << 32), "hawq_conv_expand_reduce: bad problem size");
+    const int sub = e.out_sub >= 2 ? e.out_sub : 1, hd = (e.H - 1) / sub + 1, wd = (e.W - 1) / sub + 1;
+    const long long Msrc = (long long)e.N * e.H * e.W, M = (long long)e.N * hd * wd;
+    HAWQ_REQUIRE(M > 0 && Msrc * e.Cout * 2 < (1ll << 32), "hawq_conv_expand_reduce: bad problem size");
     p.M = (int)M, p.C3 = e.Cout;
+    p.sub = sub, p.sW = e.W, p.sHW = e.H * e.W, p.dW = wd, p.dHW = hd * wd;
     p.m_id_s = e.m_id_scalar, p.e_id_s = e.e_id_scalar, p.mq = e.mq, p.eq = e.eq, p.q_hi = e.q_hi;
     p.y_lo = wi.reduce ? (r.relu && r.q_lo < 0 ? 0 : r.q_lo) : 0, p.y_hi = wi.reduce ? r.q_hi : 0;
     p.y_planar = wi.reduce ? r.out_planar : 0;
diff --git a/hawq_amd/csrc/gemm_v2.hip b/hawq_amd/csrc/gemm_v2.hip
--- a/hawq_amd/csrc/gemm_v2.hip
+++ b/hawq_amd/csrc/gemm_v2.hip
@@ -441,7 +441,7 @@
                          !a->res_no_relu && !a->res_clamp16 && (a->res_out || a->out_q) && (!a->out_q || qout_ok));
     const bool dual_ok = !dual || (a->wgt2_k128 && a->ctab_id && a->in2_bits == a->in_bits && a->w2_bits == a->w_bits && rowb2 % 128 == 0 &&
                                    (long long)a->N * a->H2 * a->W2 * rowb2 < (1ll << 31) && (long long)a->Cout * rowb2 < (1ll << 31));
-    return a->KH == 1 && a->KW == 1 && a->stride >= 1 && a->pad == 0 && (raw || (a->fast_tables != 0 && a->ctab)) && a->wgt_k128 != nullptr && !a->in_planar && epi_ok && dual_ok &&
+    return a->KH == 1 && a->KW == 1 && a->stride >= 1 && a->pad == 0 && a->out_sub < 2 && (raw || (a->fast_tables != 0 && a->ctab)) && a->wgt_k128 != nullptr && !a->in_planar && epi_ok && dual_ok &&
            ((a->in_bits == 8 && a->w_bits == 8) || nib) && rowb % 128 == 0 && a->Cout % gi.bn == 0 && (a->in_pitch == 0 || a->in_pitch == rowb) &&
            (a->out_pitch == 0 || a->out_pitch == a->Cout) && Min * rowb < (1ll << 31) && (long long)a->Cout * rowb < (1ll << 31) && M * a->Cout < (1ll << 31);
 }
diff --git a/hawq_amd/engine.py b/hawq_amd/engine.py
--- a/hawq_amd/engine.py
+++ b/hawq_amd/engine.py
@@ -15,6 +15,20 @@
 
 RES_VBITS = 20
 U16_VBITS = 17
+
+
+def out_sub_stride(readers) -> int:
+    readers = list(readers)
+    if not readers:
+        return 0
+    s = readers[0][2]
+    if s <= 1 or any((kh, kw, st, pad) != (1, 1, s, 0) for kh, kw, st, pad in readers):
+        return 0
+    return int(s)
+
+
+def out_sub_extent(n: int, s: int) -> int:
+    return (n - 1) // s + 1
 
 
 def _no_preshift(ek) -> bool:
@@ -689,20 +703,25 @@
         h, w = H1, W1
         res_bits_in = 16
         fused_in = None
+        sub_out = 0
         self._er_args, self._er_names = [], []
         for ui, u in enumerate(units):
             nxt = units[ui + 1] if ui + 1 < len(units) else None
             x_in, x_bits, hin, win, x_planar = qa, u['a_bits'], h, w, False
+            sub_in, sub_out = sub_out, 0
+            if nxt is not None and nxt['resize'] and not u['resize'] and not self.keep_acc and not os.environ.get("HAWQ_NO_OUT_SUB"):
+                sub_out = out_sub_stride((r.kh, r.kw, r.stride, r.pad) for r in (nxt['convs'][0]['conv'], nxt['ident']))
             for ci, ent in enumerate(u['convs']):
                 c = ent['conv']
+                c_stride = 1 if (sub_in and ci == 0) else c.stride
                 if ci == 0 and fused_in is not None:
                     x_in, x_bits, x_planar = fused_in
-                    hin, win = (hin + 2 * c.pad - c.kh) // c.stride + 1, (win + 2 * c.pad - c.kw) // c.stride + 1
+                    hin, win = (hin + 2 * c.pad - c.kh) // c_stride + 1, (win + 2 * c.pad - c.kw) // c_stride + 1
                     fused_in = None
                     self.n_fast += 1
                     self.n_conv += 1
                     continue
-                ho, wo = (hin + 2 * c.pad - c.kh) // c.stride + 1, (win + 2 * c.pad - c.kw) // c.stride + 1
+                ho, wo = (hin + 2 * c.pad - c.kh) // c_stride + 1, (win + 2 * c.pad - c.kw) // c_stride + 1
                 a = _lib.ConvArgs()
                 a.in_, a.wgt, a.bias = x_in.data_ptr(), c.w.data_ptr(), c.bias.data_ptr()
                 if x_bits == c.w_bits and c.band() is not None:
@@ -710,7 +729,7 @@
                 if x_bits == c.w_bits and c.k128() is not None:
                     a.wgt_k128 = c.k128().data_ptr()
                 a.N, a.H, a.W, a.Cin, a.Cout = N, hin, win, c.cin, c.cout
-                a.KH, a.KW, a.stride, a.pad = c.kh, c.kw, c.stride, c.pad
+                a.KH, a.KW, a.stride, a.pad = c.kh, c.kw, c_stride, c.pad
                 a.in_bits, a.w_bits = x_bits, c.w_bits
                 a.m, a.e = ent['m'].data_ptr(), ent['e'].data_ptr()
                 a.flags = self.flags.data_ptr()
@@ -749,7 +768,7 @@
                         a.in2, a.wgt2, a.bias2 = qa.data_ptr(), ic.w.data_ptr(), ic.bias.data_ptr()
                         if u['a_bits'] == ic.w_bits and ic.k128() is not None:
                             a.wgt2_k128 = ic.k128().data_ptr()
-                        a.H2, a.W2, a.Cin2, a.stride2 = h, w, ic.cin, ic.stride
+                        a.H2, a.W2, a.Cin2, a.stride2 = h, w, ic.cin, (1 if sub_in else ic.stride)
                         a.in2_bits, a.w2_bits = u['a_bits'], ic.w_bits
                         a.m_id, a.e_id = u['m_id'].data_ptr(), u['e_id'].data_ptr()
                     else:
@@ -757,6 +776,11 @@
                         a.m_id_scalar, a.e_id_scalar = u['m_id_s'], u['e_id_s']
                     need_res = (nxt is None) or (not nxt['resize'])
                     new_res = self._alloc(N * ho * wo * c.cout, rdt) if need_res else None
+                    if sub_out:
+                        a.out_sub = sub_out
+                        qh, qw = out_sub_extent(ho, sub_out), out_sub_extent(wo, sub_out)
+                    else:
+                        qh, qw = ho, wo
                     if new_res is not None:
                         a.res_out, a.res_out_bits = new_res.data_ptr(), self.res_bits
                         self.res_taps[u['name']] = (new_res, (N, ho, wo, c.cout))
@@ -772,7 +796,7 @@
                 keep.append(a)
                 fz = self._try_fuse(a, u, nxt, N, ho, wo, keep) if (ci == len(u['convs']) - 1 and not self.keep_acc) else None
                 if fz is None and ci == len(u['convs']) - 1 and nxt is not None:
-                    new_qa = self._alloc(N * ho * wo * c.cout * nxt['a_bits'] // 8, torch.uint8)
+                    new_qa = self._alloc(N * qh * qw * c.cout * nxt['a_bits'] // 8, torch.uint8)
                     a.out_q = new_qa.data_ptr()
                     keep.append(new_qa)
                 if fz is not None:
@@ -797,7 +821,7 @@
                 ops.append(self._conv_ops[-1])
                 if ci < len(u['convs']) - 1:
                     x_in, x_bits, hin, win, x_planar = x_next, xb_next, ho, wo, planar_next
-            res, qa, h, w = new_res, new_qa, ho, wo
+            res, qa, h, w = new_res, new_qa, qh, qw
             res_bits_in = self.res_bits
         cl = units[-1]['convs'][-1]['conv'].cout
         qf = self._alloc(N * cl, torch.int8)
diff --git a/include/hawq_mi355.h b/include/hawq_mi355.h
--- a/include/hawq_mi355.h
+++ b/include/hawq_mi355.h
@@ -61,6 +61,7 @@
     const void *wgt_band;
     const void *wgt_k128;
     const void *wgt2_k128;
+    int32_t out_sub;
 } hawq_conv_args;
 
 int hawq_conv2d(const hawq_conv_args *args, void *stream);
```

Result: faster. 106,800, median of 6 (+5.3%).
